# lucidrains/alphafold2

Measured on NVIDIA B200. Metric: evoformer_residue_pairs_per_sec, higher is better.
Workload: dtype bf16

## Files before the change

alphafold2_b200/csrc/api.cu:

```cuda
#include <cuda.h>
#include <cuda_runtime.h>
#include <cudaTypedefs.h>
#include <nvtx3/nvToolsExt.h>

#include <cstdarg>
#include <cstdio>
#include <cstdlib>
#include <cstring>
#include <vector>

#include "../../include/af2b200.h"
#include "attention_tc.cuh"
#include "chan2tok_tma.cuh"
#include "gemm_tc.cuh"
#include "ff_tc.cuh"
#include "proj_tc.cuh"
#include "simt_kernels.cuh"
#include "strict_kernels.cuh"
#include "glue_kernels.cuh"

using namespace af2;

namespace {

thread_local char g_err[512] = "";

int fail(int code, const char* fmt, ...) {
  va_list ap;
  va_start(ap, fmt);
  vsnprintf(g_err, sizeof(g_err), fmt, ap);
  va_end(ap);
  return code;
}

#define CUDA_OK(expr)                                                                            \
  do {                                                                                           \
    cudaError_t _e = (expr);                                                                     \
    if (_e != cudaSuccess) return fail(AF2_ERR_CUDA, "%s: %s (%s:%d)", #expr, cudaGetErrorString(_e), __FILE__, __LINE__); \
  } while (0)
#define AF2_TRY(expr)            \
  do {                           \
    int _r = (expr);             \
    if (_r != AF2_OK) return _r; \
  } while (0)

constexpr int MAX_DEVICES = 64;
int cur_dev() {
  int dev = 0;
  cudaGetDevice(&dev);
  return (dev >= 0 && dev < MAX_DEVICES) ? dev : 0;
}
int sm_count() {
  static int n[MAX_DEVICES] = {0};
  const int dev = cur_dev();
  if (n[dev] == 0) {
    cudaDeviceGetAttribute(&n[dev], cudaDevAttrMultiProcessorCount, dev);
    if (n[dev] <= 0) n[dev] = 148;
  }
  return n[dev];
}

int g_x_evict_last = 0;
inline int x_hint(long long tokens, int d) {
  const double mb = (double)tokens * d * 4 / 1e6;
  return (g_x_evict_last && mb >= 48.0 && mb <= 100.0) ? 1 : 0;
}

int g_pdl = 1;
template <class... KArgs, class... Args>
cudaError_t launch_pdl(void (*kern)(KArgs...), dim3 grid, dim3 block, size_t smem, cudaStream_t s, Args&&... args) {
  cudaLaunchConfig_t cfg;
  memset(&cfg, 0, sizeof(cfg));
  cfg.gridDim = grid; cfg.blockDim = block; cfg.dynamicSmemBytes = smem; cfg.stream = s;
  cudaLaunchAttribute at[1];
  at[0].id = cudaLaunchAttributeProgrammaticStreamSerialization;
  at[0].val.programmaticStreamSerializationAllowed = 1;
  cfg.attrs = at; cfg.numAttrs = g_pdl ? 1 : 0;
  return cudaLaunchKernelEx(&cfg, kern, static_cast<KArgs>(args)...);
}

struct NvtxRange {
  explicit NvtxRange(const char* name) { nvtxRangePushA(name); }
  ~NvtxRange() { nvtxRangePop(); }
};

enum KClass { KC_GEMM_LINEAR = 0, KC_GEMM_CHANNEL = 1, KC_ATTENTION = 2, KC_LAYERNORM = 3, KC_CHAN2TOK = 4, KC_MISC = 5, KC_COUNT = 6 };
struct ProfRec { cudaEvent_t a, b; int cls; double flops, bytes; };
unsigned long long g_launches = 0;
bool g_prof = false;
std::vector<ProfRec> g_recs;
std::vector<cudaEvent_t> g_pool;

cudaEvent_t prof_event() {
  if (!g_pool.empty()) { cudaEvent_t e = g_pool.back(); g_pool.pop_back(); return e; }
  cudaEvent_t e; cudaEventCreate(&e); return e;
}
struct ProfScope {
  cudaStream_t s; bool on; ProfRec r;
  ProfScope(cudaStream_t st, int cls, double flops, double bytes) : s(st), on(g_prof) {
    ++g_launches;
    if (on) { r.a = prof_event(); r.b = prof_event(); r.cls = cls; r.flops = flops; r.bytes = bytes; cudaEventRecord(r.a, s); }
  }
  ~ProfScope() { if (on) { cudaEventRecord(r.b, s); g_recs.push_back(r); } }
};

PFN_cuTensorMapEncodeTiled_v12000 encode_fn() {
  static PFN_cuTensorMapEncodeTiled_v12000 fn = nullptr;
  if (!fn) {
    void* p = nullptr;
    cudaDriverEntryPointQueryResult q;
    if (cudaGetDriverEntryPoint("cuTensorMapEncodeTiled", &p, cudaEnableDefault, &q) == cudaSuccess &&
        q == cudaDriverEntryPointSuccess)
      fn = reinterpret_cast<PFN_cuTensorMapEncodeTiled_v12000>(p);
  }
  return fn;
}

int make_tmap(CUtensorMap* m, const void* base, int rank, const unsigned long long* dims,
              const unsigned long long* strides_bytes, const unsigned* box, CUtensorMapSwizzle swz,
              CUtensorMapDataType dt = CU_TENSOR_MAP_DATA_TYPE_BFLOAT16,
              CUtensorMapL2promotion promo = CU_TENSOR_MAP_L2_PROMOTION_L2_256B) {
  auto fn = encode_fn();
  if (!fn) return fail(AF2_ERR_CUDA, "cuTensorMapEncodeTiled entry point not available");
  cuuint64_t gdim[5];
  cuuint64_t gstr[4];
  cuuint32_t bx[5], es[5];
  for (int i = 0; i < rank; ++i) {
    gdim[i] = dims[i];
    bx[i] = box[i];
    es[i] = 1;
  }
  for (int i = 0; i + 1 < rank; ++i) gstr[i] = strides_bytes[i];
  if (reinterpret_cast<uintptr_t>(base) & 15) return fail(AF2_ERR_BAD_ARG, "TMA base pointer not 16-byte aligned");
  for (int i = 0; i + 1 < rank; ++i)
    if (gstr[i] & 15) return fail(AF2_ERR_BAD_ARG, "TMA stride %d (%llu B) not a multiple of 16", i, (unsigned long long)gstr[i]);
  CUresult r = fn(m, dt, rank, const_cast<void*>(base), gdim, gstr, bx, es,
                  CU_TENSOR_MAP_INTERLEAVE_NONE, swz, promo,
                  CU_TENSOR_MAP_FLOAT_OOB_FILL_NONE);
  if (r != CUDA_SUCCESS) return fail(AF2_ERR_CUDA, "cuTensorMapEncodeTiled failed with CUresult %d", (int)r);
  return AF2_OK;
}

bool aligned16(const void* p) { return (reinterpret_cast<uintptr_t>(p) & 15) == 0; }
inline long long align_up(long long v, long long a) { return (v + a - 1) / a * a; }

struct Arena {
  char* base;
  long long size, off;
  bool ok;
  Arena(void* b, long long s) : base(static_cast<char*>(b)), size(s), off(0), ok(true) {}
  template <class T>
  T* take(long long count) {
    long long bytes = align_up(count * (long long)sizeof(T), 256);
    if (off + bytes > size) {
      ok = false;
      return nullptr;
    }
    T* p = reinterpret_cast<T*>(base + off);
    off += bytes;
    return p;
  }
};

struct GemmCall {
  const void* A; long long lda; long long a_batch;
  const void* Bm; long long ldb; long long b_batch;
  int M, N, K, batch;
  bool mn_major;
  int bn;
  int mode, act, layout, use_rowscale;
  void* out; long long ld_out; long long out_batch;
  const float* bias; const float* rowscale; const float* resid; long long ld_resid;
  int cm_inner, cm_pitch;
  int out_cols;
  int nseg; long long a_half, b_half;
  int a_pr, b_pr; long long a_piece, b_piece;
};

template <int BN, int STAGES, bool MN, int EK>
int launch_gemm_inst(const CUtensorMap& ta, const CUtensorMap& tb, const CUtensorMap& tc, const CUtensorMap& tr,
                     const GemmParams& p, cudaStream_t s) {
  using L = GemmSmem<BN, STAGES>;
  static bool configured[MAX_DEVICES] = {false};
  auto kern = gemm_tc_kernel<BN, STAGES, MN, EK>;
  if (!configured[cur_dev()]) {
    CUDA_OK(cudaFuncSetAttribute(kern, cudaFuncAttributeMaxDynamicSharedMemorySize, L::TOTAL));
    configured[cur_dev()] = true;
  }
  const int m_tiles = (p.M + GEMM_BM - 1) / GEMM_BM;
  const long long total = (long long)p.batch * m_tiles * p.num_ntiles;
  if (total <= 0) return AF2_OK;
  const int grid = (int)(total < sm_count() ? total : sm_count());
  const double flops = 2.0 * p.batch * (double)p.M * p.N * p.K;
  const double obytes = (p.tile.mode == EPI_STORE_BF16 ? 2.0 : (p.tile.mode == EPI_GATED_BF16 ? 1.0 : (p.tile.mode == EPI_RESID_F32 ? 8.0 : 4.0)));
  const double bytes = p.batch * ((double)p.M * p.K * 2 + (p.batch > 1 ? (double)p.N * p.K * 2 : 0) + (double)p.M * p.N * obytes) +
                       (p.batch > 1 ? 0 : (double)p.N * p.K * 2);
  ProfScope ps(s, p.batch > 1 ? KC_GEMM_CHANNEL : KC_GEMM_LINEAR, flops, bytes);
  CUDA_OK(launch_pdl(kern, dim3(grid), dim3(GEMM_THREADS), L::TOTAL, s, ta, tb, tc, tr, p));
  return AF2_OK;
}

int launch_gemm(const GemmCall& c, cudaStream_t s) {
  if (c.M <= 0 || c.N <= 0 || c.K <= 0 || c.batch <= 0) return AF2_OK;
  CUtensorMap ta, tb;
  const int BN = c.bn;
  if (c.nseg > 1) {
    const unsigned long long npl = c.nseg == 6 ? 3ull : 2ull;
    const unsigned long long ab = (unsigned long long)(c.batch > 1 ? c.a_batch : 0) * 2, bb_ = (unsigned long long)(c.batch > 1 ? c.b_batch : 0) * 2;
    if (!c.mn_major) {
      unsigned long long da[4] = {(unsigned long long)c.K, (unsigned long long)c.M, npl, (unsigned long long)c.batch};
      unsigned long long sa[3] = {(unsigned long long)c.lda * 2, (unsigned long long)c.a_half * 2, ab ? ab : (unsigned long long)c.a_half * 8};
      unsigned ba[4] = {64, 128, 1, 1};
      AF2_TRY(make_tmap(&ta, c.A, 4, da, sa, ba, CU_TENSOR_MAP_SWIZZLE_128B));
      unsigned long long db[4] = {(unsigned long long)c.K, (unsigned long long)c.N, npl, (unsigned long long)c.batch};
      unsigned long long sb[3] = {(unsigned long long)c.ldb * 2, (unsigned long long)c.b_half * 2, bb_ ? bb_ : (unsigned long long)c.b_half * 8};
      unsigned bx[4] = {64, (unsigned)BN, 1, 1};
      AF2_TRY(make_tmap(&tb, c.Bm, 4, db, sb, bx, CU_TENSOR_MAP_SWIZZLE_128B));
    } else {
      unsigned long long da[4] = {(unsigned long long)c.M, (unsigned long long)c.K, npl, (unsigned long long)c.batch};
      unsigned long long sa[3] = {(unsigned long long)c.lda * 2, (unsigned long long)c.a_half * 2, ab ? ab : (unsigned long long)c.a_half * 8};
      unsigned bx[4] = {64, 64, 1, 1};
      AF2_TRY(make_tmap(&ta, c.A, 4, da, sa, bx, CU_TENSOR_MAP_SWIZZLE_128B));
      unsigned long long db[4] = {(unsigned long long)c.N, (unsigned long long)c.K, npl, (unsigned long long)c.batch};
      unsigned long long sb[3] = {(unsigned long long)c.ldb * 2, (unsigned long long)c.b_half * 2, bb_ ? bb_ : (unsigned long long)c.b_half * 8};
      AF2_TRY(make_tmap(&tb, c.Bm, 4, db, sb, bx, CU_TENSOR_MAP_SWIZZLE_128B));
    }
  } else if (!c.mn_major) {
    unsigned long long da[3] = {(unsigned long long)c.K, (unsigned long long)c.M, (unsigned long long)c.batch};
    unsigned long long sa[2] = {(unsigned long long)c.lda * 2, (unsigned long long)(c.batch > 1 ? c.a_batch : c.lda * c.M) * 2};
    unsigned ba[3] = {64, 128, 1};
    AF2_TRY(make_tmap(&ta, c.A, 3, da, sa, ba, CU_TENSOR_MAP_SWIZZLE_128B));
    unsigned long long db[3] = {(unsigned long long)c.K, (unsigned long long)c.N, (unsigned long long)c.batch};
    unsigned long long sb[2] = {(unsigned long long)c.ldb * 2, (unsigned long long)(c.batch > 1 && c.b_batch ? c.b_batch : c.ldb * c.N) * 2};
    unsigned bb[3] = {64, (unsigned)BN, 1};
    AF2_TRY(make_tmap(&tb, c.Bm, 3, db, sb, bb, CU_TENSOR_MAP_SWIZZLE_128B));
  } else {
    unsigned long long da[3] = {(unsigned long long)c.M, (unsigned long long)c.K, (unsigned long long)c.batch};
    unsigned long long sa[2] = {(unsigned long long)c.lda * 2, (unsigned long long)(c.batch > 1 ? c.a_batch : c.lda * c.K) * 2};
    unsigned bx[3] = {64, 64, 1};
    AF2_TRY(make_tmap(&ta, c.A, 3, da, sa, bx, CU_TENSOR_MAP_SWIZZLE_128B));
    unsigned long long db[3] = {(unsigned long long)c.N, (unsigned long long)c.K, (unsigned long long)c.batch};
    unsigned long long sb[2] = {(unsigned long long)c.ldb * 2, (unsigned long long)(c.batch > 1 ? c.b_batch : c.ldb * c.K) * 2};
    AF2_TRY(make_tmap(&tb, c.Bm, 3, db, sb, bx, CU_TENSOR_MAP_SWIZZLE_128B));
  }
  if (c.nseg <= 1 && (c.a_pr > 0 || c.b_pr > 0)) {
    const unsigned long long bsa = (unsigned long long)(c.batch > 1 ? c.a_batch : c.lda) * 2, bsb = (unsigned long long)(c.batch > 1 ? c.b_batch : c.ldb) * 2;
    if (!c.mn_major) {
      if (c.a_pr > 0) {
        if (c.a_pr % 128 != 0) return fail(AF2_ERR_BAD_ARG, "gemm: gathered A pieces of %d rows (need a multiple of 128)", c.a_pr);
        unsigned long long da[4] = {(unsigned long long)c.K, (unsigned long long)c.a_pr, (unsigned long long)((c.M + c.a_pr - 1) / c.a_pr), (unsigned long long)c.batch};
        unsigned long long sa[3] = {(unsigned long long)c.lda * 2, (unsigned long long)c.a_piece * 2, bsa};
        unsigned ba[4] = {64, 128, 1, 1};
        AF2_TRY(make_tmap(&ta, c.A, 4, da, sa, ba, CU_TENSOR_MAP_SWIZZLE_128B));
      }
      if (c.b_pr > 0) {
        if (!((c.b_pr % BN) == 0 || (BN % c.b_pr) == 0) || c.b_pr % 8) return fail(AF2_ERR_BAD_ARG, "gemm: gathered B pieces of %d rows do not tile BN=%d", c.b_pr, BN);
        unsigned long long db[4] = {(unsigned long long)c.K, (unsigned long long)c.b_pr, (unsigned long long)((c.N + c.b_pr - 1) / c.b_pr), (unsigned long long)c.batch};
        unsigned long long sb[3] = {(unsigned long long)c.ldb * 2, (unsigned long long)c.b_piece * 2, bsb};
        unsigned bb[4] = {64, (unsigned)(c.b_pr >= BN ? BN : c.b_pr), (unsigned)(c.b_pr >= BN ? 1 : BN / c.b_pr), 1};
        AF2_TRY(make_tmap(&tb, c.Bm, 4, db, sb, bb, CU_TENSOR_MAP_SWIZZLE_128B));
      }
    } else {
      unsigned bx[4] = {64, 64, 1, 1};
      if (c.a_pr > 0) {
        if (c.a_pr % 64) return fail(AF2_ERR_BAD_ARG, "gemm: gathered MN-major A pieces of %d columns (need a multiple of 64)", c.a_pr);
        unsigned long long da[4] = {(unsigned long long)c.a_pr, (unsigned long long)c.K, (unsigned long long)((c.M + c.a_pr - 1) / c.a_pr), (unsigned long long)c.batch};
        unsigned long long sa[3] = {(unsigned long long)c.lda * 2, (unsigned long long)c.a_piece * 2, bsa};
        AF2_TRY(make_tmap(&ta, c.A, 4, da, sa, bx, CU_TENSOR_MAP_SWIZZLE_128B));
      }
      if (c.b_pr > 0) {
        if (c.b_pr % 64) return fail(AF2_ERR_BAD_ARG, "gemm: gathered MN-major B pieces of %d columns (need a multiple of 64)", c.b_pr);
        unsigned long long db[4] = {(unsigned long long)c.b_pr, (unsigned long long)c.K, (unsigned long long)((c.N + c.b_pr - 1) / c.b_pr), (unsigned long long)c.batch};
        unsigned long long sb[3] = {(unsigned long long)c.ldb * 2, (unsigned long long)c.b_piece * 2, bsb};
        AF2_TRY(make_tmap(&tb, c.Bm, 4, db, sb, bx, CU_TENSOR_MAP_SWIZZLE_128B));
      }
    }
  }
  GemmParams p;
  memset(&p, 0, sizeof(p));
  p.M = c.M; p.N = c.N; p.K = c.K; p.batch = c.batch; p.nseg = c.nseg > 1 ? c.nseg : 1;
  if (c.nseg <= 1) { p.a_pr = c.a_pr; p.b_pr = c.b_pr; }
  p.x_evict_last = (c.mode == EPI_RESID_F32) ? x_hint(c.M, c.N) : 0;
  p.num_ntiles = (c.N + BN - 1) / BN;
  p.out_cols = c.out_cols > 0 ? c.out_cols : ((c.mode == EPI_GATED_BF16) ? c.N / 2 : c.N);
  p.rowscale = c.rowscale; p.resid = c.resid; p.ld_resid = c.ld_resid;
  p.out_batch_stride = c.out_batch;
  p.cm_inner = c.cm_inner > 0 ? c.cm_inner : 1; p.cm_pitch = c.cm_pitch > 0 ? c.cm_pitch : 1;
  p.tile.mode = c.mode; p.tile.act = c.act; p.tile.layout = c.layout; p.tile.use_rowscale = c.use_rowscale;
  p.tile.out = c.out; p.tile.bias = c.bias; p.tile.ld = c.ld_out;
  const bool out_f32 = (c.mode == EPI_RESID_F32 || c.mode == EPI_STORE_F32);
  const int es = out_f32 ? 4 : 2;
  const int W = (c.mode == EPI_GATED_BF16) ? BN / 2 : BN;
  bool direct = false;
  if (!out_f32 && (W % 64) != 0) direct = true;
  if ((reinterpret_cast<uintptr_t>(c.out) & 15) != 0) direct = true;
  if (c.layout == LAYOUT_TOKEN) {
    if ((c.ld_out * es) % 16 != 0) direct = true;
    if (c.batch > 1 && (c.out_batch * es) % 16 != 0) direct = true;
  } else {
    if (c.cm_pitch != c.cm_inner || (c.ld_out * 2) % 16 != 0 || c.batch != 1 || out_f32) direct = true;
  }
  if (c.mode == EPI_RESID_F32 && ((c.ld_resid * 4) % 16 != 0 || (reinterpret_cast<uintptr_t>(c.resid) & 15) != 0)) direct = true;
  const bool resid_w = !direct && c.mode == EPI_RESID_F32 && BN == 256 && !c.mn_major && c.batch == 1 && c.N <= 256 &&
                       p.out_cols == 256;
  CUtensorMap tc = ta, tr = ta;
  if (!direct) {
    const CUtensorMapDataType dt = out_f32 ? CU_TENSOR_MAP_DATA_TYPE_FLOAT32 : CU_TENSOR_MAP_DATA_TYPE_BFLOAT16;
    if (c.layout == LAYOUT_TOKEN) {
      unsigned long long dc[3] = {(unsigned long long)p.out_cols, (unsigned long long)c.M, (unsigned long long)c.batch};
      unsigned long long sc[2] = {(unsigned long long)c.ld_out * es, (unsigned long long)(c.batch > 1 ? c.out_batch : c.ld_out * c.M) * es};
      unsigned bc[3] = {(unsigned)(out_f32 ? 32 : 64), (unsigned)(resid_w ? 32 : 128), 1};
      AF2_TRY(make_tmap(&tc, c.out, 3, dc, sc, bc, CU_TENSOR_MAP_SWIZZLE_128B, dt));
      if (c.mode == EPI_RESID_F32) {
        unsigned long long sr[2] = {(unsigned long long)c.ld_resid * 4, (unsigned long long)c.ld_resid * c.M * 4};
        AF2_TRY(make_tmap(&tr, c.resid, 3, dc, sr, bc, CU_TENSOR_MAP_SWIZZLE_128B, dt));
      }
    } else {
      unsigned long long dc[3] = {(unsigned long long)c.M, (unsigned long long)p.out_cols, 1ull};
      unsigned long long sc[2] = {(unsigned long long)c.ld_out * 2, (unsigned long long)c.ld_out * p.out_cols * 2};
      unsigned bc[3] = {64, 64, 1};
      AF2_TRY(make_tmap(&tc, c.out, 3, dc, sc, bc, CU_TENSOR_MAP_SWIZZLE_128B, dt));
    }
  }
  p.direct = direct ? 1 : 0;
  int ek = EK_GENERIC;
  if (!direct && BN == 256) {
    if (c.mode == EPI_STORE_BF16 && c.layout == LAYOUT_TOKEN && c.act == ACT_NONE && !c.use_rowscale) ek = EK_STORE_TOK;
    else if (c.mode == EPI_STORE_BF16 && c.layout == LAYOUT_TOKEN && c.act == ACT_SIGMOID && !c.use_rowscale) ek = EK_STORE_TOK_SIG;
    else if (c.mode == EPI_STORE_BF16 && c.layout == LAYOUT_CHANNEL && c.act == ACT_NONE) ek = EK_STORE_CH;
    else if (c.mode == EPI_GATED_BF16 && c.layout == LAYOUT_TOKEN && c.act == ACT_GELU && !c.use_rowscale) ek = EK_GATED_TOK_GELU;
    else if (c.mode == EPI_GATED_BF16 && c.layout == LAYOUT_CHANNEL && c.act == ACT_SIGMOID) ek = EK_GATED_CH_SIG;
    else if (c.mode == EPI_RESID_F32) ek = resid_w ? EK_RESID_F32_W : EK_RESID_F32;
    else if (c.mode == EPI_STORE_F32) ek = EK_STORE_F32;
  }
  if (c.mn_major) {
    if (BN == 256) {
      if (ek == EK_STORE_F32) return launch_gemm_inst<256, 3, true, EK_STORE_F32>(ta, tb, tc, tr, p, s);
      return launch_gemm_inst<256, 3, true, EK_GENERIC>(ta, tb, tc, tr, p, s);
    }
    if (BN == 128) return launch_gemm_inst<128, 4, true, EK_GENERIC>(ta, tb, tc, tr, p, s);
    return launch_gemm_inst<64, 6, true, EK_GENERIC>(ta, tb, tc, tr, p, s);
  }
  if (BN == 256) {
    switch (ek) {
      case EK_STORE_TOK: return launch_gemm_inst<256, 3, false, EK_STORE_TOK>(ta, tb, tc, tr, p, s);
      case EK_STORE_TOK_SIG: return launch_gemm_inst<256, 3, false, EK_STORE_TOK_SIG>(ta, tb, tc, tr, p, s);
      case EK_STORE_CH: return launch_gemm_inst<256, 3, false, EK_STORE_CH>(ta, tb, tc, tr, p, s);
      case EK_GATED_TOK_GELU: return launch_gemm_inst<256, 3, false, EK_GATED_TOK_GELU>(ta, tb, tc, tr, p, s);
      case EK_GATED_CH_SIG: return launch_gemm_inst<256, 3, false, EK_GATED_CH_SIG>(ta, tb, tc, tr, p, s);
      case EK_RESID_F32: return launch_gemm_inst<256, 3, false, EK_RESID_F32>(ta, tb, tc, tr, p, s);
      case EK_RESID_F32_W: return launch_gemm_inst<256, 3, false, EK_RESID_F32_W>(ta, tb, tc, tr, p, s);
      case EK_STORE_F32: return launch_gemm_inst<256, 3, false, EK_STORE_F32>(ta, tb, tc, tr, p, s);
      default: return launch_gemm_inst<256, 3, false, EK_GENERIC>(ta, tb, tc, tr, p, s);
    }
  }
  if (BN == 128) return launch_gemm_inst<128, 4, false, EK_GENERIC>(ta, tb, tc, tr, p, s);
  return launch_gemm_inst<64, 6, false, EK_GENERIC>(ta, tb, tc, tr, p, s);
}

int pick_bn(int n) { return n > 128 ? 256 : (n > 64 ? 128 : 64); }

GemmCall linear_call(const void* A, long long lda, const void* W, long long ldw, int M, int N, int K) {
  GemmCall c;
  memset(&c, 0, sizeof(c));
  c.A = A; c.lda = lda; c.Bm = W; c.ldb = ldw; c.M = M; c.N = N; c.K = K; c.batch = 1;
  c.mn_major = false; c.bn = pick_bn(N);
  return c;
}

int launch_layernorm(const LnParams& p, cudaStream_t s) {
  if (p.T <= 0) return AF2_OK;
  if (p.d % 4 != 0 || p.d > 1024) return fail(AF2_ERR_BAD_ARG, "LayerNorm: dim %d must be a multiple of 4 and <= 1024", p.d);
  const long long blocks_needed = (p.T + 7) / 8;
  const long long cap = (long long)sm_count() * 16;
  const int grid = (int)(blocks_needed < cap ? blocks_needed : cap);
  ProfScope ps(s, KC_LAYERNORM, 0.0, (double)p.T * p.d * (p.y ? 6.0 : 4.0) + (p.wb ? (double)p.T * p.heads * 2 : 0));
  if (p.d <= 128) layernorm_rows_kernel<1><<<grid, 256, 0, s>>>(p);
  else if (p.d <= 256) layernorm_rows_kernel<2><<<grid, 256, 0, s>>>(p);
  else if (p.d <= 512) layernorm_rows_kernel<4><<<grid, 256, 0, s>>>(p);
  else layernorm_rows_kernel<8><<<grid, 256, 0, s>>>(p);
  CUDA_OK(cudaGetLastError());
  return AF2_OK;
}

bool pair_bias_fast_ok(int d, int heads) { return d % 32 == 0 && d >= 32 && d <= 256 && heads <= 8; }
int launch_pair_bias(const float* x, long long T, int d, const float* wb, __nv_bfloat16* bias_out, int heads, long long bias_hs,
                     int n_inner, int pitch, cudaStream_t s, int transpose = 0) {
  if (T <= 0) return AF2_OK;
  PairBiasParams p;
  p.x = x; p.T = T; p.d = d; p.wb = wb; p.bias_out = bias_out; p.heads = heads; p.bias_hs = bias_hs; p.n_inner = n_inner; p.pitch = pitch;
  p.x_evict_last = x_hint(T, d);
  p.transpose = transpose;
  if (T > 0x7fffffffLL) return fail(AF2_ERR_BAD_ARG, "pair_bias: too many tokens");
  const bool mma = (d == 256 || d == 128);
  const long long need = mma ? (T + 127) / 128 : (T + 31) / 32;
  const long long cap = (long long)sm_count() * 3;
  const int grid = (int)(need < cap ? need : cap);
  ProfScope ps(s, KC_LAYERNORM, 0.0, (double)T * d * 4 + (double)T * heads * 2);
  if (mma && d == 256) CUDA_OK(launch_pdl(pair_bias_mma_kernel<16>, dim3(grid), dim3(256), 0, s, p));
  else if (mma) CUDA_OK(launch_pdl(pair_bias_mma_kernel<8>, dim3(grid), dim3(256), 0, s, p));
  else {
    switch (d / 32) {
      case 7: pair_bias_kernel<7><<<grid, 256, 0, s>>>(p); break;
      case 6: pair_bias_kernel<6><<<grid, 256, 0, s>>>(p); break;
      case 5: pair_bias_kernel<5><<<grid, 256, 0, s>>>(p); break;
      case 3: pair_bias_kernel<3><<<grid, 256, 0, s>>>(p); break;
      case 2: pair_bias_kernel<2><<<grid, 256, 0, s>>>(p); break;
      default: pair_bias_kernel<1><<<grid, 256, 0, s>>>(p); break;
    }
  }
  CUDA_OK(cudaGetLastError());
  return AF2_OK;
}

template <int D>
int launch_chan_to_token_tma(const ChanLnParams& p, long long T, cudaStream_t s) {
  using L = Chan2TokSmem<D>;
  static bool configured[MAX_DEVICES] = {false};
  auto kern = chan_to_token_tma_kernel<D>;
  if (!configured[cur_dev()]) {
    CUDA_OK(cudaFuncSetAttribute(kern, cudaFuncAttributeMaxDynamicSharedMemorySize, L::TOTAL));
    configured[cur_dev()] = true;
  }
  CUtensorMap tx, tg, ty;
  {
    unsigned long long dx[2] = {(unsigned long long)T, (unsigned long long)D};
    unsigned long long sx[1] = {(unsigned long long)p.chan_stride * 4};
    unsigned bx[2] = {C2T_TOK, (unsigned)D};
    AF2_TRY(make_tmap(&tx, p.src, 2, dx, sx, bx, CU_TENSOR_MAP_SWIZZLE_NONE, CU_TENSOR_MAP_DATA_TYPE_FLOAT32));
    unsigned long long dy[2] = {(unsigned long long)D, (unsigned long long)T};
    unsigned long long sy[1] = {(unsigned long long)D * 2};
    unsigned by[2] = {64, C2T_TOK};
    AF2_TRY(make_tmap(&ty, p.y, 2, dy, sy, by, CU_TENSOR_MAP_SWIZZLE_128B));
    if (p.mode == 0) AF2_TRY(make_tmap(&tg, p.gate, 2, dy, sy, by, CU_TENSOR_MAP_SWIZZLE_128B));
    else tg = ty;
  }
  Chan2TokParams q;
  q.T = T; q.mode = p.mode; q.gamma = p.gamma; q.beta = p.beta; q.scale = p.scale; q.scale_const = p.scale_const; q.eps = p.eps;
  const long long tiles = (T + C2T_TOK - 1) / C2T_TOK;
  const int grid = (int)(tiles < sm_count() ? tiles : sm_count());
  ProfScope ps(s, KC_CHAN2TOK, 0.0, (double)T * D * (p.mode == 0 ? 8.0 : 6.0));
  CUDA_OK(launch_pdl(kern, dim3(grid), dim3(L::THREADS), L::TOTAL, s, tx, tg, ty, q));
  return AF2_OK;
}

int g_c2t_tma = 1;
int g_attn_bias_t = 0;
int g_attn_ident_tmem = 1;
int g_attn_skip = 0;
int g_attn_k3 = 0;
int g_attn_headmajor = 0;
long long* g_attn_trace = nullptr;
int g_attn_l2pf = 0;
int g_attn_group = 1;
int g_gather_fused = 1;

int launch_chan_to_token(const ChanLnParams& p, cudaStream_t s) {
  const long long T = (long long)p.rows * p.n;
  if (g_c2t_tma && p.pitch == p.n && (p.d == 256 || p.d == 128) && (p.chan_stride % 4) == 0 && T > 0 && T < (1ll << 31) &&
      aligned16(p.src) && aligned16(p.y) && (p.mode != 0 || aligned16(p.gate))) {
    return p.d == 256 ? launch_chan_to_token_tma<256>(p, T, s) : launch_chan_to_token_tma<128>(p, T, s);
  }
  if (p.pitch == p.n && p.d % 64 == 0 && p.d <= 256 && (T % 4) == 0) {
    const size_t smem = (size_t)p.d * 64 * sizeof(float) + 8 * 64 * 2 * sizeof(float);
    static bool configured[MAX_DEVICES] = {false};
    if (!configured[cur_dev()]) {
      CUDA_OK(cudaFuncSetAttribute(chan_to_token_tile_kernel<32>, cudaFuncAttributeMaxDynamicSharedMemorySize, 256 * 64 * 4 + 4096));
      CUDA_OK(cudaFuncSetAttribute(chan_to_token_tile_kernel<24>, cudaFuncAttributeMaxDynamicSharedMemorySize, 192 * 64 * 4 + 4096));
      configured[cur_dev()] = true;
    }
    ProfScope ps(s, KC_CHAN2TOK, 0.0, (double)T * p.d * (p.mode == 0 ? 8.0 : 6.0));
    const unsigned grid = (unsigned)((T + 63) / 64);
    switch (p.d / 64) {
      case 4: chan_to_token_tile_kernel<32><<<grid, 512, smem, s>>>(p, T); break;
      case 3: chan_to_token_tile_kernel<24><<<grid, 512, smem, s>>>(p, T); break;
      case 2: chan_to_token_tile_kernel<16><<<grid, 512, smem, s>>>(p, T); break;
      default: chan_to_token_tile_kernel<8><<<grid, 512, smem, s>>>(p, T); break;
    }
    CUDA_OK(cudaGetLastError());
    return AF2_OK;
  }
  const size_t smem = (size_t)p.d * 33 * sizeof(float);
  static size_t configured[MAX_DEVICES] = {0};
  if (smem > 48 * 1024 && smem > configured[cur_dev()]) {
    CUDA_OK(cudaFuncSetAttribute(chan_to_token_kernel, cudaFuncAttributeMaxDynamicSharedMemorySize, (int)smem));
    configured[cur_dev()] = smem;
  }
  dim3 grid((p.n + 31) / 32, p.rows);
  ProfScope ps(s, KC_CHAN2TOK, 0.0, (double)p.rows * p.n * p.d * (p.mode == 0 ? 8.0 : 6.0));
  chan_to_token_kernel<<<grid, 256, smem, s>>>(p);
  CUDA_OK(cudaGetLastError());
  return AF2_OK;
}

template <int DH>
int launch_attention_inst(const CUtensorMap& tq, const CUtensorMap& tk, const CUtensorMap& tv, const CUtensorMap& tbias,
                          const CUtensorMap& tg, const CUtensorMap& to, const AttnParams& p, cudaStream_t s) {
  using L = AttnSmem<DH>;
  static bool configured[MAX_DEVICES] = {false};
  auto kern = attention_tc_kernel<DH>;
  if (!configured[cur_dev()]) {
    CUDA_OK(cudaFuncSetAttribute(kern, cudaFuncAttributeMaxDynamicSharedMemorySize, L::TOTAL));
    configured[cur_dev()] = true;
  }
  const int nqb = (p.n + 127) / 128;
  const long long items = (long long)nqb * p.heads * p.nbatch;
  if (items <= 0) return AF2_OK;
  int grid = (int)(items < sm_count() ? items : sm_count());
  if (nqb >= 2 && nqb <= 8 && g_attn_group) grid = grid / nqb * nqb;
  const double tokens = (double)p.n * p.nbatch;
  ProfScope ps(s, KC_ATTENTION, 4.0 * tokens * p.n * p.heads * DH,
               tokens * p.heads * DH * 2.0 * 5 + (p.has_bias ? (double)p.heads * p.n * p.n * 2 : 0));
  CUDA_OK(launch_pdl(kern, dim3(grid), dim3(ATTN_THREADS), L::TOTAL, s, tq, tk, tv, tbias, tg, to, p));
  return AF2_OK;
}

int launch_attention(const __nv_bfloat16* qkv, int heads, int dh, int n, int nbatch, long long tok_sb, long long tok_si,
                     const __nv_bfloat16* bias, int npad, const uint8_t* mask, const __nv_bfloat16* gate,
                     __nv_bfloat16* out, cudaStream_t s, const __nv_bfloat16* qkv_hm = nullptr, long long hm_tokens = 0, int bias_t = 0) {
  const long long I = (long long)heads * dh;
  const long long ld = 3 * I;
  CUtensorMap tq, tk, tv, tb, tg, to;
  unsigned long long dims[4] = {(unsigned long long)dh, (unsigned long long)n, (unsigned long long)heads, (unsigned long long)nbatch};
  unsigned long long str[3] = {(unsigned long long)(tok_si * ld * 2), (unsigned long long)(dh * 2), (unsigned long long)(tok_sb * ld * 2)};
  if (qkv_hm) {
    str[0] = (unsigned long long)(tok_si * dh * 2); str[1] = (unsigned long long)(hm_tokens * dh * 2); str[2] = (unsigned long long)(tok_sb * dh * 2);
  }
  unsigned box[4] = {(unsigned)dh, 128, 1, 1};
  const CUtensorMapSwizzle swz = (dh == 64) ? CU_TENSOR_MAP_SWIZZLE_128B : CU_TENSOR_MAP_SWIZZLE_64B;
  const CUtensorMapL2promotion promo = (dh == 64) ? CU_TENSOR_MAP_L2_PROMOTION_L2_128B : CU_TENSOR_MAP_L2_PROMOTION_L2_64B;
  const CUtensorMapDataType bf = CU_TENSOR_MAP_DATA_TYPE_BFLOAT16;
  if (qkv_hm) {
    const long long part = (long long)heads * hm_tokens * dh;
    AF2_TRY(make_tmap(&tq, qkv_hm, 4, dims, str, box, swz, bf, CU_TENSOR_MAP_L2_PROMOTION_L2_256B));
    AF2_TRY(make_tmap(&tk, qkv_hm + part, 4, dims, str, box, swz, bf, CU_TENSOR_MAP_L2_PROMOTION_L2_256B));
    AF2_TRY(make_tmap(&tv, qkv_hm + 2 * part, 4, dims, str, box, swz, bf, CU_TENSOR_MAP_L2_PROMOTION_L2_256B));
  } else {
    AF2_TRY(make_tmap(&tq, qkv, 4, dims, str, box, swz, bf, promo));
    AF2_TRY(make_tmap(&tk, qkv + I, 4, dims, str, box, swz, bf, promo));
    AF2_TRY(make_tmap(&tv, qkv + 2 * I, 4, dims, str, box, swz, bf, promo));
  }
  unsigned long long gstr[3] = {(unsigned long long)(tok_si * I * 2), (unsigned long long)(dh * 2), (unsigned long long)(tok_sb * I * 2)};
  AF2_TRY(make_tmap(&tg, gate, 4, dims, gstr, box, swz, bf, promo));
  unsigned obox[4] = {(unsigned)dh, 32, 1, 1};
  AF2_TRY(make_tmap(&to, out, 4, dims, gstr, obox, swz));
  if (bias) {
    unsigned long long bd[3] = {(unsigned long long)npad, (unsigned long long)n, (unsigned long long)heads};
    unsigned long long bs[2] = {(unsigned long long)npad * 2, (unsigned long long)n * npad * 2};
    unsigned bb[3] = {64, 128, 1};
    AF2_TRY(make_tmap(&tb, bias, 3, bd, bs, bb, CU_TENSOR_MAP_SWIZZLE_128B));
  } else {
    tb = tq;
  }
  AttnParams p;
  memset(&p, 0, sizeof(p));
  p.n = n; p.heads = heads; p.nbatch = nbatch; p.has_bias = bias != nullptr;
  p.mask = mask; p.mask_sb = tok_sb; p.mask_si = tok_si;
  p.gate = gate; p.out = out; p.tok_sb = tok_sb; p.tok_si = tok_si; p.ld_gate = I; p.ld_out = I;
  p.l2_prefetch = g_attn_l2pf;
  p.k_stages3 = g_attn_k3;
  p.dbg_skip = g_attn_skip;
  p.ident_tmem = g_attn_ident_tmem;
  p.bias_t = bias_t;
  p.trace = g_attn_trace;
  if (dh == 64) return launch_attention_inst<64>(tq, tk, tv, tb, tg, to, p, s);
  if (dh == 32) return launch_attention_inst<32>(tq, tk, tv, tb, tg, to, p, s);
  return fail(AF2_ERR_BAD_ARG, "attention: dim_head %d unsupported (32 or 64)", dh);
}

#include "proj_launch.inl"

int g_ff_fused = 1;

bool ff_fused_ok(const af2_ff_weights* w, int d, int hidden) {
  return g_ff_fused && g_proj_ctas == 2 && w->w_cat && w->w_ext && w->bn == 256 && (d == 128 || d == 256) &&
         hidden % FF_CHUNK == 0 && aligned16(w->w2) && aligned16(w->b2);
}

int launch_ff_fused(const af2_ff_weights* w, float* x, long long T, int d, int hidden, cudaStream_t s) {
  if (T <= 0) return AF2_OK;
  if (!aligned16(x)) return fail(AF2_ERR_BAD_ARG, "feed_forward: x not 16-byte aligned");
  using L = FfSmem;
  static bool configured_dev[MAX_DEVICES] = {false};
  static int max_clusters_dev[MAX_DEVICES] = {0};
  int& max_clusters = max_clusters_dev[cur_dev()];
  if (!configured_dev[cur_dev()]) {
    CUDA_OK(cudaFuncSetAttribute(ff_tc_kernel, cudaFuncAttributeMaxDynamicSharedMemorySize, L::TOTAL));
    cudaLaunchConfig_t qc;
    memset(&qc, 0, sizeof(qc));
    qc.gridDim = dim3(sm_count(), 1, 1); qc.blockDim = dim3(FF_THREADS, 1, 1); qc.dynamicSmemBytes = L::TOTAL;
    cudaLaunchAttribute qa[1];
    qa[0].id = cudaLaunchAttributeClusterDimension; qa[0].val.clusterDim.x = 2; qa[0].val.clusterDim.y = 1; qa[0].val.clusterDim.z = 1;
    qc.attrs = qa; qc.numAttrs = 1;
    int nc = 0;
    if (cudaOccupancyMaxActiveClusters(&nc, ff_tc_kernel, &qc) != cudaSuccess || nc <= 0) { cudaGetLastError(); nc = sm_count() / 2; }
    max_clusters = nc < sm_count() / 2 ? nc : sm_count() / 2;
    configured_dev[cur_dev()] = true;
  }
  const int n1p = (hidden + 127) / 128 * 256;
  CUtensorMap tw1, tb1, tw2, tx;
  {
    unsigned long long dw[2] = {(unsigned long long)d, (unsigned long long)n1p};
    unsigned long long sw[1] = {(unsigned long long)d * 2};
    unsigned bw[2] = {64, 64};
    AF2_TRY(make_tmap(&tw1, w->w_cat, 2, dw, sw, bw, CU_TENSOR_MAP_SWIZZLE_128B));
    unsigned long long dx[2] = {16ull, (unsigned long long)n1p};
    unsigned long long sx[1] = {32ull};
    unsigned bx[2] = {16, 64};
    AF2_TRY(make_tmap(&tb1, w->w_ext, 2, dx, sx, bx, CU_TENSOR_MAP_SWIZZLE_32B));
    unsigned long long d2[2] = {(unsigned long long)hidden, (unsigned long long)d};
    unsigned long long s2[1] = {(unsigned long long)hidden * 2};
    unsigned b2[2] = {64, (unsigned)(d / 2)};
    AF2_TRY(make_tmap(&tw2, w->w2, 2, d2, s2, b2, CU_TENSOR_MAP_SWIZZLE_128B));
    unsigned long long dxr[2] = {(unsigned long long)d, (unsigned long long)T};
    unsigned long long sxr[1] = {(unsigned long long)d * 4};
    unsigned bxr[2] = {32, 32};
    AF2_TRY(make_tmap(&tx, x, 2, dxr, sxr, bxr, CU_TENSOR_MAP_SWIZZLE_128B, CU_TENSOR_MAP_DATA_TYPE_FLOAT32));
  }
  FfParams p;
  memset(&p, 0, sizeof(p));
  p.x = x; p.b2 = w->b2; p.T = T; p.d = d; p.hidden = hidden; p.inv_d = 1.0f / (float)d; p.eps = 1e-5f;
  p.m_units = (int)((T + 255) / 256);
  const int clusters = p.m_units < max_clusters ? p.m_units : max_clusters;
  const double flops = 2.0 * T * (double)d * hidden * 3;
  const double bytes = (double)T * d * 8 + (double)n1p * d * 2 + (double)d * hidden * 2;
  ProfScope ps(s, KC_GEMM_LINEAR, flops, bytes);
  cudaLaunchConfig_t cfg;
  memset(&cfg, 0, sizeof(cfg));
  cfg.gridDim = dim3(clusters * 2, 1, 1); cfg.blockDim = dim3(FF_THREADS, 1, 1); cfg.dynamicSmemBytes = L::TOTAL; cfg.stream = s;
  cudaLaunchAttribute at[2];
  at[0].id = cudaLaunchAttributeClusterDimension; at[0].val.clusterDim.x = 2; at[0].val.clusterDim.y = 1; at[0].val.clusterDim.z = 1;
  at[1].id = cudaLaunchAttributeProgrammaticStreamSerialization; at[1].val.programmaticStreamSerializationAllowed = 1;
  cfg.attrs = at; cfg.numAttrs = g_pdl ? 2 : 1;
  CUDA_OK(cudaLaunchKernelEx(&cfg, ff_tc_kernel, tw1, tb1, tw2, tx, p));
  return AF2_OK;
}

int launch_outer_scale(const uint8_t* mask, float* scale, uint32_t* words, int row0, int rows, int S, int N, float eps, cudaStream_t s);

int ew_grid(long long n) {
  long long b = (n + 255) / 256;
  long long cap = (long long)sm_count() * 8;
  return (int)(b < cap ? (b > 0 ? b : 1) : cap);
}

int launch_outer_scale(const uint8_t* mask, float* scale, uint32_t* words, int row0, int rows, int S, int N, float eps, cudaStream_t s) {
  const long long T = (long long)rows * N;
  if (T <= 0) return AF2_OK;
  const int nw = (S + 31) / 32;
  const size_t smem = (size_t)nw * N * 4;
  ProfScope ps(s, KC_MISC, 0.0, 0.0);
  if (words && smem <= 160 * 1024) {
    static size_t configured[MAX_DEVICES] = {0};
    if (smem > 48 * 1024 && smem > configured[cur_dev()]) {
      CUDA_OK(cudaFuncSetAttribute(outer_scale_bits_kernel, cudaFuncAttributeMaxDynamicSharedMemorySize, (int)smem));
      configured[cur_dev()] = smem;
    }
    mask_pack_bits_kernel<<<ew_grid((long long)nw * N), 256, 0, s>>>(mask, words, S, N);
    CUDA_OK(cudaGetLastError());
    const long long need = (T + 255) / 256;
    const int grid = (int)(need < sm_count() ? need : sm_count());
    outer_scale_bits_kernel<<<grid, 256, smem, s>>>(words, scale, row0, rows, S, N, eps);
  } else {
    outer_scale_rows_kernel<<<ew_grid(T), 256, 0, s>>>(mask, scale, row0, rows, S, N, eps);
  }
  CUDA_OK(cudaGetLastError());
  return AF2_OK;
}

}

extern "C" {

const char* af2_last_error(void) { return g_err; }
int af2_abi_version(void) { return 2; }

unsigned long long af2_launch_count(void) { return g_launches; }

void af2_profile_enable(int on) {
  g_prof = on != 0;
  if (g_prof) {
    for (auto& r : g_recs) { g_pool.push_back(r.a); g_pool.push_back(r.b); }
    g_recs.clear();
  }
}

long long af2_profile_read(int cls, double* ms, double* flops, double* bytes) {
  cudaDeviceSynchronize();
  double t = 0, f = 0, b = 0;
  long long n = 0;
  for (auto& r : g_recs) {
    if (r.cls != cls) continue;
    float e = 0.f;
    if (cudaEventElapsedTime(&e, r.a, r.b) == cudaSuccess) t += e;
    f += r.flops; b += r.bytes; ++n;
  }
  if (ms) *ms = t;
  if (flops) *flops = f;
  if (bytes) *bytes = b;
  return n;
}

int af2_debug_proj_trace(long long* out) {
  if (!g_proj_trace) return fail(AF2_ERR_BAD_ARG, "projection trace not enabled (AF2_PROJ_TRACE=1)");
  CUDA_OK(cudaDeviceSynchronize());
  CUDA_OK(cudaMemcpy(out, g_proj_trace, 2048 * sizeof(long long), cudaMemcpyDeviceToHost));
  return AF2_OK;
}

int af2_debug_attn_trace(long long* out) {
  if (!g_attn_trace) return fail(AF2_ERR_BAD_ARG, "attention trace not enabled (AF2_ATTN_TRACE=1)");
  CUDA_OK(cudaDeviceSynchronize());
  CUDA_OK(cudaMemcpy(out, g_attn_trace, 1024 * sizeof(long long), cudaMemcpyDeviceToHost));
  CUDA_OK(cudaMemset(g_attn_trace, 0, 1024 * sizeof(long long)));
  return AF2_OK;
}

void af2_set_proj_mode(int ctas) { g_proj_ctas = ctas < 0 ? 2 : (ctas > 2 ? 2 : ctas); }
void af2_set_ff_fused(int on) { g_ff_fused = on != 0; }

int af2_check_device(void) {
  if (const char* e = getenv("AF2_PROJ_CTAS")) af2_set_proj_mode(atoi(e));
  if (const char* e = getenv("AF2_FF_FUSED")) af2_set_ff_fused(atoi(e));
  if (const char* e = getenv("AF2_C2T_TMA")) g_c2t_tma = atoi(e) != 0;
  if (const char* e = getenv("AF2_PROJ_PRODTILES")) g_proj_prod_tiles = atof(e);
  if (const char* e = getenv("AF2_PROJ_BALANCE")) g_proj_balance = atoi(e) != 0;
  if (const char* e = getenv("AF2_PROJ_WIDE")) g_proj_wide = atoi(e) != 0;
  if (const char* e = getenv("AF2_PROJ_L2PF")) g_proj_l2pf = atoi(e) != 0;
  if (const char* e = getenv("AF2_GATHER_FUSED")) g_gather_fused = atoi(e) != 0;
  if (const char* e = getenv("AF2_ATTN_GROUP")) g_attn_group = atoi(e) != 0;
  if (const char* e = getenv("AF2_ATTN_L2PF")) g_attn_l2pf = atoi(e) != 0;
  if (const char* e = getenv("AF2_ATTN_HEADMAJOR")) g_attn_headmajor = atoi(e) != 0;
  if (const char* e = getenv("AF2_ATTN_K3")) g_attn_k3 = atoi(e) != 0;
  if (const char* e = getenv("AF2_ATTN_SKIP")) g_attn_skip = atoi(e);
  if (const char* e = getenv("AF2_ATTN_IDENT_TMEM")) g_attn_ident_tmem = atoi(e) != 0;
  if (const char* e = getenv("AF2_ATTN_BIAS_T")) g_attn_bias_t = atoi(e) != 0;
  if (const char* e = getenv("AF2_ATTN_TRACE")) {
    if (atoi(e) != 0 && !g_attn_trace) {
      if (cudaMalloc(&g_attn_trace, 1024 * sizeof(long long)) != cudaSuccess) g_attn_trace = nullptr;
      else cudaMemset(g_attn_trace, 0, 1024 * sizeof(long long));
    }
  }
  if (const char* e = getenv("AF2_X_EVICT_LAST")) g_x_evict_last = atoi(e) != 0;
  if (const char* e = getenv("AF2_PDL")) g_pdl = atoi(e) != 0;
  if (const char* e = getenv("AF2_PROJ_TRACE")) {
    if (atoi(e) != 0 && !g_proj_trace) {
      if (cudaMalloc(&g_proj_trace, 2048 * sizeof(long long)) != cudaSuccess) g_proj_trace = nullptr;
      else cudaMemset(g_proj_trace, 0, 2048 * sizeof(long long));
    }
  }
  int dev = 0;
  if (cudaGetDevice(&dev) != cudaSuccess) return fail(AF2_ERR_CUDA, "no CUDA device");
  int major = 0;
  cudaDeviceGetAttribute(&major, cudaDevAttrComputeCapabilityMajor, dev);
  if (major != 10) return fail(AF2_ERR_UNSUPPORTED_DEVICE, "libaf2b200 is built for sm_100a only; device has compute capability %d.x", major);
  return AF2_OK;
}

long long af2_feed_forward_workspace(long long tokens, int d, int hidden) {
  return align_up(tokens * d * 2, 256) + align_up(tokens * hidden * 2, 256) + 1024;
}

int af2_feed_forward(const af2_ff_weights* w, float* x, long long tokens, int d, int hidden, void* workspace,
                     long long workspace_bytes, af2_stream_t stream) {
  NvtxRange nvtx_("af2_feed_forward");
  cudaStream_t s = static_cast<cudaStream_t>(stream);
  if (!w || !x) return fail(AF2_ERR_BAD_ARG, "feed_forward: null argument");
  if (d % 8 || hidden % 8) return fail(AF2_ERR_BAD_ARG, "feed_forward: d=%d and hidden=%d must be multiples of 8", d, hidden);
  if (tokens > 0x7fffffffLL) return fail(AF2_ERR_BAD_ARG, "feed_forward: too many tokens");
  if (ff_fused_ok(w, d, hidden)) return launch_ff_fused(w, x, tokens, d, hidden, s);
  Arena ar(workspace, workspace_bytes);
  __nv_bfloat16* xn = ar.take<__nv_bfloat16>(tokens * d);
  __nv_bfloat16* hbuf = ar.take<__nv_bfloat16>(tokens * hidden);
  if (!ar.ok) return fail(AF2_ERR_WORKSPACE, "feed_forward: workspace too small");
  const int half = w->bn / 2;
  const int n1p = (hidden + half - 1) / half * w->bn;
  if (g_proj_ctas > 0 && w->w_cat && w->bn == 256 && proj_dim_ok(d)) {
    ProjCall pc;
    memset(&pc, 0, sizeof(pc));
    pc.x = x; pc.T = tokens; pc.d = d;
    pc.w_cat = w->w_cat; pc.w_ext = w->w_ext; pc.nseg = 1;
    pc.seg[0] = ProjOut{n1p / 256, EK_GATED_TOK_GELU, hidden, hbuf, hidden};
    AF2_TRY(launch_proj(pc, s));
  } else {
    LnParams lp;
    memset(&lp, 0, sizeof(lp));
    lp.x = x; lp.gamma = w->ln_gamma; lp.beta = w->ln_beta; lp.y = xn; lp.T = tokens; lp.d = d; lp.eps = 1e-5f;
    AF2_TRY(launch_layernorm(lp, s));
    GemmCall c1 = linear_call(xn, d, w->w1, d, (int)tokens, n1p, d);
    c1.bn = w->bn; c1.mode = EPI_GATED_BF16; c1.act = ACT_GELU; c1.layout = LAYOUT_TOKEN;
    c1.out = hbuf; c1.ld_out = hidden; c1.bias = w->b1; c1.out_cols = hidden;
    AF2_TRY(launch_gemm(c1, s));
  }
  GemmCall c2 = linear_call(hbuf, hidden, w->w2, hidden, (int)tokens, d, hidden);
  c2.mode = EPI_RESID_F32; c2.out = x; c2.ld_out = d; c2.bias = w->b2; c2.resid = x; c2.ld_resid = d;
  AF2_TRY(launch_gemm(c2, s));
  return AF2_OK;
}

long long af2_axial_attention_workspace(int B, int h, int wdim, int d, int heads, int dim_head, int row_attn) {
  const long long T = (long long)B * h * wdim, I = (long long)heads * dim_head;
  const int n = row_attn ? wdim : h;
  const long long npad = align_up(n, 8);
  return align_up(T * d * 2, 256) + 2 * align_up(T * 3 * I * 2, 256) + 2 * align_up(T * I * 2, 256) +
         align_up((long long)B * heads * n * npad * 2, 256) + 1024;
}

static int axial_attention_impl(const af2_attn_weights* w, float* x, const float* edges, const void* pre_bias,
                                const unsigned char* mask, int B, int h, int wdim, int d, int heads, int dim_head,
                                int row_attn, void* workspace, long long workspace_bytes, af2_stream_t stream, int tied = 0) {
  NvtxRange nvtx_(row_attn ? "af2_axial_attention(row)" : "af2_axial_attention(col)");
  cudaStream_t s = static_cast<cudaStream_t>(stream);
  if (!w || !x) return fail(AF2_ERR_BAD_ARG, "axial_attention: null argument");
  if (dim_head != 32 && dim_head != 64) return fail(AF2_ERR_BAD_ARG, "axial_attention: dim_head %d unsupported (32 or 64)", dim_head);
  if (d % 8) return fail(AF2_ERR_BAD_ARG, "axial_attention: dim %d must be a multiple of 8", d);
  const long long T = (long long)B * h * wdim, I = (long long)heads * dim_head;
  if (T > 0x7fffffffLL) return fail(AF2_ERR_BAD_ARG, "axial_attention: too many tokens");
  const int n = row_attn ? wdim : h;
  const int nb = row_attn ? h : wdim;
  const int npad = (int)align_up(n, 8);
  const bool has_bias = pre_bias != nullptr || (edges != nullptr && w->w_edge != nullptr);
  Arena ar(workspace, workspace_bytes);
  __nv_bfloat16* xn = ar.take<__nv_bfloat16>(T * d);
  __nv_bfloat16* qkv = ar.take<__nv_bfloat16>(T * 3 * I);
  __nv_bfloat16* gate = ar.take<__nv_bfloat16>(T * I);
  __nv_bfloat16* og = ar.take<__nv_bfloat16>(T * I);
  __nv_bfloat16* bias = ar.take<__nv_bfloat16>((long long)B * heads * n * npad);
  __nv_bfloat16* qkv_hm = ar.take<__nv_bfloat16>(T * 3 * I);
  if (!ar.ok) return fail(AF2_ERR_WORKSPACE, "axial_attention: workspace too small");
  if (pre_bias) bias = const_cast<__nv_bfloat16*>(static_cast<const __nv_bfloat16*>(pre_bias));

  const bool fused_proj = g_proj_ctas > 0 && w->w_cat && proj_dim_ok(d) && (I % 8) == 0;
  LnParams lp;
  memset(&lp, 0, sizeof(lp));
  lp.x = x; lp.gamma = w->ln_gamma; lp.beta = w->ln_beta; lp.y = xn; lp.T = T; lp.d = d; lp.eps = 1e-5f;
  const bool fuse_bias = has_bias && !pre_bias && edges == x && B == 1;
  const bool bias_t = g_attn_bias_t && has_bias && !pre_bias && pair_bias_fast_ok(d, heads) && !(fuse_bias && !fused_proj);
  if (has_bias && !pre_bias && npad != n) CUDA_OK(cudaMemsetAsync(bias, 0, (size_t)B * heads * n * npad * 2, s));
  if (fuse_bias) {
    lp.wb = w->w_edge; lp.bias_out = bias; lp.heads = heads; lp.bias_hs = (long long)n * npad; lp.n_inner = n; lp.pitch = npad;
  }
  if (!fused_proj) {
    AF2_TRY(launch_layernorm(lp, s));
  } else if (fuse_bias) {
    if (pair_bias_fast_ok(d, heads)) {
      AF2_TRY(launch_pair_bias(x, T, d, w->w_edge, bias, heads, (long long)n * npad, n, npad, s, bias_t ? 1 : 0));
    } else {
      lp.y = nullptr;
      AF2_TRY(launch_layernorm(lp, s));
    }
  }
  if (has_bias && !fuse_bias && !pre_bias && pair_bias_fast_ok(d, heads)) {
    for (int b = 0; b < B; ++b)
      AF2_TRY(launch_pair_bias(edges + (long long)b * n * n * d, (long long)n * n, d, w->w_edge, bias + (long long)b * heads * n * npad,
                               heads, (long long)n * npad, n, npad, s, bias_t ? 1 : 0));
  } else if (has_bias && !fuse_bias && !pre_bias) {
    for (int b = 0; b < B; ++b) {
      LnParams bp;
      memset(&bp, 0, sizeof(bp));
      bp.x = edges + (long long)b * n * n * d; bp.T = (long long)n * n; bp.d = d; bp.eps = 1e-5f;
      bp.wb = w->w_edge; bp.bias_out = bias + (long long)b * heads * n * npad; bp.heads = heads;
      bp.bias_hs = (long long)n * npad; bp.n_inner = n; bp.pitch = npad;
      AF2_TRY(launch_layernorm(bp, s));
    }
  }
  if (fused_proj) {
    ProjCall pc;
    memset(&pc, 0, sizeof(pc));
    pc.x = x; pc.T = T; pc.d = d;
    pc.w_cat = w->w_cat; pc.w_ext = w->w_ext; pc.nseg = 2;
    pc.seg[0] = ProjOut{(int)((3 * I + 255) / 256), EK_STORE_TOK, (int)(3 * I), qkv, 3 * I};
    pc.seg[1] = ProjOut{(int)((I + 255) / 256), EK_STORE_TOK_SIG, (int)I, gate, I};
    AF2_TRY(launch_proj(pc, s));
  } else {
    GemmCall cq = linear_call(xn, d, w->w_qkv, d, (int)T, (int)(3 * I), d);
    cq.mode = EPI_STORE_BF16; cq.layout = LAYOUT_TOKEN; cq.out = qkv; cq.ld_out = 3 * I;
    AF2_TRY(launch_gemm(cq, s));
    GemmCall cg = linear_call(xn, d, w->w_gate, d, (int)T, (int)I, d);
    cg.mode = EPI_STORE_BF16; cg.act = ACT_SIGMOID; cg.layout = LAYOUT_TOKEN; cg.out = gate; cg.ld_out = I; cg.bias = w->b_gate;
    AF2_TRY(launch_gemm(cg, s));
  }
  const long long tok_sb = row_attn ? wdim : 1, tok_si = row_attn ? 1 : wdim;
  for (int b = 0; b < B; ++b) {
    const long long t0 = (long long)b * h * wdim;
    if (tied) {
      ProfScope ps(s, KC_MISC, 0.0, 0.0);
      tie_queries_kernel<__nv_bfloat16><<<ew_grid((long long)n * I), 256, 0, s>>>(qkv + t0 * 3 * I, 3 * I, (int)I, n, nb, tok_sb, tok_si);
      CUDA_OK(cudaGetLastError());
    }
    const long long Tb = (long long)h * wdim;
    if (g_attn_headmajor && dim_head % 8 == 0) {
      ProfScope ps(s, KC_MISC, 0.0, 0.0);
      qkv_to_headmajor_kernel<<<ew_grid(Tb * 3 * I / 8), 256, 0, s>>>(reinterpret_cast<const uint4*>(qkv + t0 * 3 * I),
                                                                        reinterpret_cast<uint4*>(qkv_hm + t0 * 3 * I), Tb, (int)(3 * I), dim_head);
      CUDA_OK(cudaGetLastError());
    }
    AF2_TRY(launch_attention(qkv + t0 * 3 * I, heads, dim_head, n, nb, tok_sb, tok_si,
                             has_bias ? bias + (long long)b * heads * n * npad : nullptr, npad,
                             mask ? mask + t0 : nullptr, gate + t0 * I, og + t0 * I, s,
                             (g_attn_headmajor && dim_head % 8 == 0) ? qkv_hm + t0 * 3 * I : nullptr, Tb, bias_t ? 1 : 0));
  }
  GemmCall co = linear_call(og, I, w->w_out, I, (int)T, d, (int)I);
  co.mode = EPI_RESID_F32; co.out = x; co.ld_out = d; co.bias = w->b_out; co.resid = x; co.ld_resid = d;
  AF2_TRY(launch_gemm(co, s));
  return AF2_OK;
}

long long af2_triangle_multiply_workspace(int B, int N, int d) {
  const long long T = (long long)B * N * N;
  const long long np8 = align_up(N, 8), np4 = align_up(N, 4);
  return 3 * align_up(T * d * 2, 256)
         + 2 * align_up((long long)d * B * N * np8 * 2, 256)
         + align_up((long long)d * B * N * np4 * 4, 256)
         + align_up(T * 4, 256) + 1024;
}

int af2_triangle_multiply(const af2_trimul_weights* w, float* x, const unsigned char* mask, int B, int N, int d,
                          int ingoing, void* workspace, long long workspace_bytes, af2_stream_t stream) {
  NvtxRange nvtx_("af2_triangle_multiply");
  cudaStream_t s = static_cast<cudaStream_t>(stream);
  if (!w || !x) return fail(AF2_ERR_BAD_ARG, "triangle_multiply: null argument");
  if (d % 32) return fail(AF2_ERR_BAD_ARG, "triangle_multiply: dim %d must be a multiple of 32", d);
  const long long T = (long long)B * N * N;
  if (T > 0x7fffffffLL) return fail(AF2_ERR_BAD_ARG, "triangle_multiply: too many tokens");
  const int np8 = (int)align_up(N, 8), np4 = (int)align_up(N, 4);
  const long long cs_lr = (long long)B * N * np8;
  const long long cs_o = (long long)B * N * np4;
  Arena ar(workspace, workspace_bytes);
  __nv_bfloat16* xn = ar.take<__nv_bfloat16>(T * d);
  __nv_bfloat16* gate = ar.take<__nv_bfloat16>(T * d);
  __nv_bfloat16* tn = ar.take<__nv_bfloat16>(T * d);
  __nv_bfloat16* Lc = ar.take<__nv_bfloat16>(d * cs_lr);
  __nv_bfloat16* Rc = ar.take<__nv_bfloat16>(d * cs_lr);
  float* Oc = ar.take<float>(d * cs_o);
  float* maskf = ar.take<float>(T);
  if (!ar.ok) return fail(AF2_ERR_WORKSPACE, "triangle_multiply: workspace too small");

  const bool fused_front = g_proj_ctas > 0 && w->w_cat && w->bn == 256 && proj_dim_ok(d) && np8 == N;
  if (fused_front) {
    ProjCall pc;
    memset(&pc, 0, sizeof(pc));
    pc.x = x; pc.T = T; pc.d = d;
    pc.w_cat = w->w_cat; pc.w_ext = w->w_ext; pc.rowmask = mask; pc.nseg = 3;
    const int tl = (d + 127) / 128;
    pc.seg[0] = ProjOut{tl, EK_GATED_CH_SIG, d, Lc, cs_lr};
    pc.seg[1] = ProjOut{tl, EK_GATED_CH_SIG, d, Rc, cs_lr};
    pc.seg[2] = ProjOut{(d + 255) / 256, EK_STORE_TOK_SIG, d, gate, (long long)d};
    AF2_TRY(launch_proj(pc, s));
  }
  LnParams lp;
  memset(&lp, 0, sizeof(lp));
  lp.x = x; lp.gamma = w->ln_gamma; lp.beta = w->ln_beta; lp.y = xn; lp.T = T; lp.d = d; lp.eps = 1e-5f;
  if (!fused_front) AF2_TRY(launch_layernorm(lp, s));
  if (mask && !fused_front) {
    { ProfScope ps(s, KC_MISC, 0.0, 0.0); mask_to_float_kernel<<<ew_grid(T), 256, 0, s>>>(mask, maskf, T); }
    CUDA_OK(cudaGetLastError());
  }
  if (np8 != N) {
    CUDA_OK(cudaMemsetAsync(Lc, 0, (size_t)d * cs_lr * 2, s));
    CUDA_OK(cudaMemsetAsync(Rc, 0, (size_t)d * cs_lr * 2, s));
  }
  const int half = w->bn / 2;
  const int npk = (d + half - 1) / half * w->bn;
  for (int side = 0; side < 2 && !fused_front; ++side) {
    GemmCall c = linear_call(xn, d, side ? w->w_right : w->w_left, d, (int)T, npk, d);
    c.bn = w->bn; c.mode = EPI_GATED_BF16; c.act = ACT_SIGMOID; c.layout = LAYOUT_CHANNEL;
    c.out = side ? Rc : Lc; c.ld_out = cs_lr; c.bias = side ? w->b_right : w->b_left;
    c.use_rowscale = mask != nullptr; c.rowscale = maskf; c.cm_inner = N; c.cm_pitch = np8; c.out_cols = d;
    AF2_TRY(launch_gemm(c, s));
  }
  GemmCall cg = linear_call(xn, d, w->w_ogate, d, (int)T, d, d);
  cg.mode = EPI_STORE_BF16; cg.act = ACT_SIGMOID; cg.layout = LAYOUT_TOKEN; cg.out = gate; cg.ld_out = d; cg.bias = w->b_ogate;
  if (!fused_front) AF2_TRY(launch_gemm(cg, s));
  for (int b = 0; b < B; ++b) {
    GemmCall c;
    memset(&c, 0, sizeof(c));
    const long long boff = (long long)b * N * np8;
    if (!ingoing) {
      c.A = Lc + boff; c.Bm = Rc + boff; c.mn_major = false;
    } else {
      c.A = Rc + boff; c.Bm = Lc + boff; c.mn_major = true;
    }
    c.lda = np8; c.ldb = np8; c.a_batch = cs_lr; c.b_batch = cs_lr;
    c.M = N; c.N = N; c.K = N; c.batch = d; c.bn = pick_bn(N);
    c.mode = EPI_STORE_F32; c.layout = LAYOUT_TOKEN; c.out = Oc + (long long)b * N * np4; c.ld_out = np4; c.out_batch = cs_o;
    AF2_TRY(launch_gemm(c, s));
  }
  ChanLnParams cp;
  memset(&cp, 0, sizeof(cp));
  cp.src = Oc; cp.chan_stride = cs_o; cp.pitch = np4; cp.rows = B * N; cp.n = N; cp.d = d; cp.mode = 0;
  cp.gamma = w->on_gamma; cp.beta = w->on_beta; cp.gate = gate; cp.eps = 1e-5f; cp.y = tn;
  AF2_TRY(launch_chan_to_token(cp, s));
  GemmCall co = linear_call(tn, d, w->w_out, d, (int)T, d, d);
  co.mode = EPI_RESID_F32; co.out = x; co.ld_out = d; co.bias = w->b_out; co.resid = x; co.ld_resid = d;
  AF2_TRY(launch_gemm(co, s));
  return AF2_OK;
}

long long af2_outer_mean_workspace(int B, int S, int N, int d) {
  const long long Tm = (long long)B * S * N, Tx = (long long)B * N * N;
  const long long np8 = align_up(N, 8), np4 = align_up(N, 4);
  return align_up(Tm * d * 2, 256) + align_up((long long)2 * d * B * S * np8 * 2, 256) +
         align_up((long long)d * B * N * np4 * 4, 256) + align_up(Tx * d * 2, 256) + align_up(Tm * 4, 256) +
         align_up(Tx * 4, 256) + align_up((long long)((S + 31) / 32) * N * 4, 256) + 1024;
}

int af2_outer_mean(const af2_outer_weights* w, float* x, const float* m, const unsigned char* msa_mask, int B, int S,
                   int N, int d, float eps, void* workspace, long long workspace_bytes, af2_stream_t stream) {
  NvtxRange nvtx_("af2_outer_mean");
  cudaStream_t s = static_cast<cudaStream_t>(stream);
  if (!w || !x || !m) return fail(AF2_ERR_BAD_ARG, "outer_mean: null argument");
  if (d % 32) return fail(AF2_ERR_BAD_ARG, "outer_mean: dim %d must be a multiple of 32", d);
  const long long Tm = (long long)B * S * N, Tx = (long long)B * N * N;
  if (Tm > 0x7fffffffLL || Tx > 0x7fffffffLL) return fail(AF2_ERR_BAD_ARG, "outer_mean: too many tokens");
  const int np8 = (int)align_up(N, 8), np4 = (int)align_up(N, 4);
  const long long cs_lr = (long long)B * S * np8, cs_o = (long long)B * N * np4;
  Arena ar(workspace, workspace_bytes);
  __nv_bfloat16* mn = ar.take<__nv_bfloat16>(Tm * d);
  __nv_bfloat16* LRc = ar.take<__nv_bfloat16>(2LL * d * cs_lr);
  float* Oc = ar.take<float>(d * cs_o);
  __nv_bfloat16* tn = ar.take<__nv_bfloat16>(Tx * d);
  float* maskf = ar.take<float>(Tm);
  float* scale = ar.take<float>(Tx);
  uint32_t* mwords = ar.take<uint32_t>((long long)((S + 31) / 32) * N);
  if (!ar.ok) return fail(AF2_ERR_WORKSPACE, "outer_mean: workspace too small");

  const bool fused_front = g_proj_ctas > 0 && w->w_cat && proj_dim_ok(d) && np8 == N;
  LnParams lp;
  memset(&lp, 0, sizeof(lp));
  lp.x = m; lp.gamma = w->ln_gamma; lp.beta = w->ln_beta; lp.y = mn; lp.T = Tm; lp.d = d; lp.eps = 1e-5f;
  if (!fused_front) AF2_TRY(launch_layernorm(lp, s));
  if (msa_mask) {
    if (!fused_front) { ProfScope ps(s, KC_MISC, 0.0, 0.0); mask_to_float_kernel<<<ew_grid(Tm), 256, 0, s>>>(msa_mask, maskf, Tm); }
    CUDA_OK(cudaGetLastError());
    for (int b = 0; b < B; ++b)
      AF2_TRY(launch_outer_scale(msa_mask + (long long)b * S * N, scale + (long long)b * N * N, mwords, 0, N, S, N, eps, s));
  }
  if (np8 != N) CUDA_OK(cudaMemsetAsync(LRc, 0, (size_t)2 * d * cs_lr * 2, s));
  if (fused_front) {
    ProjCall pc;
    memset(&pc, 0, sizeof(pc));
    pc.x = m; pc.T = Tm; pc.d = d;
    pc.w_cat = w->w_cat; pc.w_ext = w->w_ext; pc.rowmask = msa_mask; pc.nseg = 1;
    pc.seg[0] = ProjOut{(2 * d + 255) / 256, EK_STORE_CH, 2 * d, LRc, cs_lr};
    AF2_TRY(launch_proj(pc, s));
  } else {
    GemmCall c = linear_call(mn, d, w->w_lr, d, (int)Tm, 2 * d, d);
    c.mode = EPI_STORE_BF16; c.layout = LAYOUT_CHANNEL; c.out = LRc; c.ld_out = cs_lr; c.bias = w->b_lr;
    c.use_rowscale = msa_mask != nullptr; c.rowscale = maskf; c.cm_inner = N; c.cm_pitch = np8;
    AF2_TRY(launch_gemm(c, s));
  }
  for (int b = 0; b < B; ++b) {
    GemmCall g;
    memset(&g, 0, sizeof(g));
    g.A = LRc + (long long)b * S * np8; g.Bm = LRc + (long long)d * cs_lr + (long long)b * S * np8;
    g.mn_major = true; g.lda = np8; g.ldb = np8; g.a_batch = cs_lr; g.b_batch = cs_lr;
    g.M = N; g.N = N; g.K = S; g.batch = d; g.bn = pick_bn(N);
    g.mode = EPI_STORE_F32; g.layout = LAYOUT_TOKEN; g.out = Oc + (long long)b * N * np4; g.ld_out = np4; g.out_batch = cs_o;
    AF2_TRY(launch_gemm(g, s));
  }
  ChanLnParams cp;
  memset(&cp, 0, sizeof(cp));
  cp.src = Oc; cp.chan_stride = cs_o; cp.pitch = np4; cp.rows = B * N; cp.n = N; cp.d = d; cp.mode = 1;
  cp.scale = msa_mask ? scale : nullptr; cp.scale_const = 1.0f / (float)S; cp.y = tn;
  AF2_TRY(launch_chan_to_token(cp, s));
  GemmCall co = linear_call(tn, d, w->w_out, d, (int)Tx, d, d);
  co.mode = EPI_RESID_F32; co.out = x; co.ld_out = d; co.bias = w->b_out; co.resid = x; co.ld_resid = d;
  AF2_TRY(launch_gemm(co, s));
  return AF2_OK;
}


int af2_axial_attention(const af2_attn_weights* w, float* x, const float* edges, const unsigned char* mask, int B,
                        int h, int wdim, int d, int heads, int dim_head, int row_attn, void* workspace,
                        long long workspace_bytes, af2_stream_t stream) {
  return axial_attention_impl(w, x, edges, nullptr, mask, B, h, wdim, d, heads, dim_head, row_attn, workspace,
                              workspace_bytes, stream);
}

int af2_axial_attention_ex(const af2_attn_weights* w, float* x, const float* edges, const unsigned char* mask, int B,
                           int h, int wdim, int d, int heads, int dim_head, int row_attn, int flags, void* workspace,
                           long long workspace_bytes, af2_stream_t stream) {
  return axial_attention_impl(w, x, edges, nullptr, mask, B, h, wdim, d, heads, dim_head, row_attn, workspace,
                              workspace_bytes, stream, flags & 1);
}

int af2_axial_attention_prebias(const af2_attn_weights* w, float* x, const void* bias_bf16, const unsigned char* mask,
                                int B, int h, int wdim, int d, int heads, int dim_head, int row_attn, void* workspace,
                                long long workspace_bytes, af2_stream_t stream) {
  return axial_attention_impl(w, x, nullptr, bias_bf16, mask, B, h, wdim, d, heads, dim_head, row_attn, workspace,
                              workspace_bytes, stream);
}

int af2_pair_bias(const float* x_rows, const float* w_edge, void* bias_out, int rows, int n, int d, int heads,
                  af2_stream_t stream) {
  NvtxRange nvtx_("af2_pair_bias");
  cudaStream_t s = static_cast<cudaStream_t>(stream);
  if (!x_rows || !w_edge || !bias_out) return fail(AF2_ERR_BAD_ARG, "pair_bias: null argument");
  const int npad = (int)align_up(n, 8);
  if (pair_bias_fast_ok(d, heads))
    return launch_pair_bias(x_rows, (long long)rows * n, d, w_edge, static_cast<__nv_bfloat16*>(bias_out), heads, (long long)rows * npad,
                            n, npad, s);
  LnParams bp;
  memset(&bp, 0, sizeof(bp));
  bp.x = x_rows; bp.T = (long long)rows * n; bp.d = d; bp.eps = 1e-5f;
  bp.wb = w_edge; bp.bias_out = static_cast<__nv_bfloat16*>(bias_out); bp.heads = heads;
  bp.bias_hs = (long long)rows * npad; bp.n_inner = n; bp.pitch = npad;
  return launch_layernorm(bp, s);
}

long long af2_triangle_project_workspace(long long tokens, int d) {
  return align_up(tokens * d * 2, 256) + align_up(tokens * 4, 256) + 1024;
}

int af2_triangle_project(const af2_trimul_weights* w, const float* x, const unsigned char* mask, long long tokens,
                         int inner, int d, void* Lc, void* Rc, long long chan_stride, void* gate, void* workspace,
                         long long workspace_bytes, af2_stream_t stream) {
  NvtxRange nvtx_("af2_triangle_project");
  cudaStream_t s = static_cast<cudaStream_t>(stream);
  if (!w || !x || !Lc || !Rc || !gate) return fail(AF2_ERR_BAD_ARG, "triangle_project: null argument");
  if (d % 32) return fail(AF2_ERR_BAD_ARG, "triangle_project: dim %d must be a multiple of 32", d);
  if (tokens % inner) return fail(AF2_ERR_BAD_ARG, "triangle_project: tokens must be a multiple of inner");
  const int pitch = (int)align_up(inner, 8);
  Arena ar(workspace, workspace_bytes);
  __nv_bfloat16* xn = ar.take<__nv_bfloat16>(tokens * d);
  float* maskf = ar.take<float>(tokens);
  if (!ar.ok) return fail(AF2_ERR_WORKSPACE, "triangle_project: workspace too small");
  if (g_proj_ctas > 0 && w->w_cat && w->bn == 256 && proj_dim_ok(d) && pitch == inner) {
    ProjCall pc;
    memset(&pc, 0, sizeof(pc));
    pc.x = x; pc.T = tokens; pc.d = d;
    pc.w_cat = w->w_cat; pc.w_ext = w->w_ext; pc.rowmask = mask; pc.nseg = 3;
    const int tl = (d + 127) / 128;
    pc.seg[0] = ProjOut{tl, EK_GATED_CH_SIG, d, Lc, chan_stride};
    pc.seg[1] = ProjOut{tl, EK_GATED_CH_SIG, d, Rc, chan_stride};
    pc.seg[2] = ProjOut{(d + 255) / 256, EK_STORE_TOK_SIG, d, gate, (long long)d};
    return launch_proj(pc, s);
  }
  LnParams lp;
  memset(&lp, 0, sizeof(lp));
  lp.x = x; lp.gamma = w->ln_gamma; lp.beta = w->ln_beta; lp.y = xn; lp.T = tokens; lp.d = d; lp.eps = 1e-5f;
  AF2_TRY(launch_layernorm(lp, s));
  if (mask) {
    { ProfScope ps(s, KC_MISC, 0.0, 0.0); mask_to_float_kernel<<<ew_grid(tokens), 256, 0, s>>>(mask, maskf, tokens); }
    CUDA_OK(cudaGetLastError());
  }
  if (pitch != inner) {
    CUDA_OK(cudaMemsetAsync(Lc, 0, (size_t)d * chan_stride * 2, s));
    CUDA_OK(cudaMemsetAsync(Rc, 0, (size_t)d * chan_stride * 2, s));
  }
  const int half = w->bn / 2;
  const int npk = (d + half - 1) / half * w->bn;
  for (int side = 0; side < 2; ++side) {
    GemmCall c = linear_call(xn, d, side ? w->w_right : w->w_left, d, (int)tokens, npk, d);
    c.bn = w->bn; c.mode = EPI_GATED_BF16; c.act = ACT_SIGMOID; c.layout = LAYOUT_CHANNEL;
    c.out = side ? Rc : Lc; c.ld_out = chan_stride; c.bias = side ? w->b_right : w->b_left;
    c.use_rowscale = mask != nullptr; c.rowscale = maskf; c.cm_inner = inner; c.cm_pitch = pitch; c.out_cols = d;
    AF2_TRY(launch_gemm(c, s));
  }
  GemmCall cg = linear_call(xn, d, w->w_ogate, d, (int)tokens, d, d);
  cg.mode = EPI_STORE_BF16; cg.act = ACT_SIGMOID; cg.layout = LAYOUT_TOKEN; cg.out = gate; cg.ld_out = d; cg.bias = w->b_ogate;
  AF2_TRY(launch_gemm(cg, s));
  return AF2_OK;
}

long long af2_triangle_contract_workspace(int rows, int cols, int d) {
  return align_up((long long)d * rows * align_up(cols, 4) * 4, 256) + align_up((long long)rows * cols * d * 2, 256) + 1024;
}

int af2_triangle_contract(const af2_trimul_weights* w, float* x, const void* Lc, long long cs_l, const void* Rg,
                          long long cs_r, long long piece_stride, int pieces, const void* gate, int rows, int cols,
                          int K, int d, int ingoing, void* workspace, long long workspace_bytes, af2_stream_t stream) {
  NvtxRange nvtx_("af2_triangle_contract");
  cudaStream_t s = static_cast<cudaStream_t>(stream);
  if (!w || !x || !Lc || !Rg || !gate || pieces < 1) return fail(AF2_ERR_BAD_ARG, "triangle_contract: bad argument");
  if ((!ingoing && cols % pieces) || (ingoing && rows % pieces)) return fail(AF2_ERR_BAD_ARG, "triangle_contract: pieces must divide the gathered axis");
  const long long T = (long long)rows * cols;
  const int cp4 = (int)align_up(cols, 4);
  const long long cs_o = (long long)rows * cp4;
  Arena ar(workspace, workspace_bytes);
  float* Oc = ar.take<float>(d * cs_o);
  __nv_bfloat16* tn = ar.take<__nv_bfloat16>(T * d);
  if (!ar.ok) return fail(AF2_ERR_WORKSPACE, "triangle_contract: workspace too small");
  const __nv_bfloat16* L = static_cast<const __nv_bfloat16*>(Lc);
  const __nv_bfloat16* R = static_cast<const __nv_bfloat16*>(Rg);
  bool fused_pieces = false;
  if (pieces > 1 && g_gather_fused) {
    GemmCall c;
    memset(&c, 0, sizeof(c));
    c.batch = d; c.K = K; c.mode = EPI_STORE_F32; c.layout = LAYOUT_TOKEN; c.ld_out = cp4; c.out_batch = cs_o; c.out = Oc;
    if (!ingoing) {
      const int pc = cols / pieces, bn = pick_bn(cols);
      if (pc % 8 == 0 && (pc % bn == 0 || bn % pc == 0)) {
        c.A = L; c.lda = align_up(K, 8); c.a_batch = cs_l;
        c.Bm = R; c.ldb = align_up(K, 8); c.b_batch = cs_r; c.b_pr = pc; c.b_piece = piece_stride;
        c.mn_major = false; c.M = rows; c.N = cols; c.bn = bn;
        fused_pieces = true;
      }
    } else {
      const int pr = rows / pieces;
      if (pr % 64 == 0) {
        c.A = R; c.lda = align_up(pr, 8); c.a_batch = cs_r; c.a_pr = pr; c.a_piece = piece_stride;
        c.Bm = L; c.ldb = align_up(cols, 8); c.b_batch = cs_l;
        c.mn_major = true; c.M = rows; c.N = cols; c.bn = pick_bn(cols);
        fused_pieces = true;
      }
    }
    if (fused_pieces) AF2_TRY(launch_gemm(c, s));
  }
  for (int p = 0; p < pieces && !fused_pieces; ++p) {
    GemmCall c;
    memset(&c, 0, sizeof(c));
    c.batch = d; c.K = K; c.mode = EPI_STORE_F32; c.layout = LAYOUT_TOKEN; c.ld_out = cp4; c.out_batch = cs_o;
    if (!ingoing) {
      const int pc = cols / pieces;
      c.A = L; c.lda = align_up(K, 8); c.a_batch = cs_l;
      c.Bm = R + p * piece_stride; c.ldb = align_up(K, 8); c.b_batch = cs_r;
      c.mn_major = false; c.M = rows; c.N = pc; c.bn = pick_bn(pc);
      c.out = Oc + (long long)p * pc;
    } else {
      const int pr = rows / pieces;
      c.A = R + p * piece_stride; c.lda = align_up(pr, 8); c.a_batch = cs_r;
      c.Bm = L; c.ldb = align_up(cols, 8); c.b_batch = cs_l;
      c.mn_major = true; c.M = pr; c.N = cols; c.bn = pick_bn(cols);
      c.out = Oc + (long long)p * pr * cp4;
    }
    AF2_TRY(launch_gemm(c, s));
  }
  ChanLnParams cp;
  memset(&cp, 0, sizeof(cp));
  cp.src = Oc; cp.chan_stride = cs_o; cp.pitch = cp4; cp.rows = rows; cp.n = cols; cp.d = d; cp.mode = 0;
  cp.gamma = w->on_gamma; cp.beta = w->on_beta; cp.gate = static_cast<const __nv_bfloat16*>(gate); cp.eps = 1e-5f; cp.y = tn;
  AF2_TRY(launch_chan_to_token(cp, s));
  GemmCall co = linear_call(tn, d, w->w_out, d, (int)T, d, d);
  co.mode = EPI_RESID_F32; co.out = x; co.ld_out = d; co.bias = w->b_out; co.resid = x; co.ld_resid = d;
  AF2_TRY(launch_gemm(co, s));
  return AF2_OK;
}

long long af2_outer_project_workspace(long long tokens, int d) {
  return align_up(tokens * d * 2, 256) + align_up(tokens * 4, 256) + 1024;
}

int af2_outer_project(const af2_outer_weights* w, const float* m, const unsigned char* msa_mask, long long tokens,
                      int inner, int d, void* LRc, long long chan_stride, void* workspace, long long workspace_bytes,
                      af2_stream_t stream) {
  NvtxRange nvtx_("af2_outer_project");
  cudaStream_t s = static_cast<cudaStream_t>(stream);
  if (!w || !m || !LRc) return fail(AF2_ERR_BAD_ARG, "outer_project: null argument");
  if (d % 32) return fail(AF2_ERR_BAD_ARG, "outer_project: dim %d must be a multiple of 32", d);
  const int pitch = (int)align_up(inner, 8);
  Arena ar(workspace, workspace_bytes);
  __nv_bfloat16* mn = ar.take<__nv_bfloat16>(tokens * d);
  float* maskf = ar.take<float>(tokens);
  if (!ar.ok) return fail(AF2_ERR_WORKSPACE, "outer_project: workspace too small");
  if (g_proj_ctas > 0 && w->w_cat && proj_dim_ok(d) && pitch == inner) {
    ProjCall pc;
    memset(&pc, 0, sizeof(pc));
    pc.x = m; pc.T = tokens; pc.d = d;
    pc.w_cat = w->w_cat; pc.w_ext = w->w_ext; pc.rowmask = msa_mask; pc.nseg = 1;
    pc.seg[0] = ProjOut{(2 * d + 255) / 256, EK_STORE_CH, 2 * d, LRc, chan_stride};
    return launch_proj(pc, s);
  }
  LnParams lp;
  memset(&lp, 0, sizeof(lp));
  lp.x = m; lp.gamma = w->ln_gamma; lp.beta = w->ln_beta; lp.y = mn; lp.T = tokens; lp.d = d; lp.eps = 1e-5f;
  AF2_TRY(launch_layernorm(lp, s));
  if (msa_mask) {
    { ProfScope ps(s, KC_MISC, 0.0, 0.0); mask_to_float_kernel<<<ew_grid(tokens), 256, 0, s>>>(msa_mask, maskf, tokens); }
    CUDA_OK(cudaGetLastError());
  }
  if (pitch != inner) CUDA_OK(cudaMemsetAsync(LRc, 0, (size_t)2 * d * chan_stride * 2, s));
  GemmCall c = linear_call(mn, d, w->w_lr, d, (int)tokens, 2 * d, d);
  c.mode = EPI_STORE_BF16; c.layout = LAYOUT_CHANNEL; c.out = LRc; c.ld_out = chan_stride; c.bias = w->b_lr;
  c.use_rowscale = msa_mask != nullptr; c.rowscale = maskf; c.cm_inner = inner; c.cm_pitch = pitch;
  AF2_TRY(launch_gemm(c, s));
  return AF2_OK;
}

long long af2_outer_contract_workspace(int rows, int N, int d) {
  return align_up((long long)d * rows * align_up(N, 4) * 4, 256) + align_up((long long)rows * N * d * 2, 256) +
         align_up((long long)rows * N * 4, 256) + align_up((long long)N * 4096 / 8, 256) + 1024;
}

int af2_outer_contract(const af2_outer_weights* w, float* x, const void* Lc, long long cs_l, const void* Rg,
                       long long cs_r, long long piece_stride, int pieces, const unsigned char* msa_mask_full,
                       int row0, int rows, int N, int S, int d, float eps, void* workspace, long long workspace_bytes,
                       af2_stream_t stream) {
  NvtxRange nvtx_("af2_outer_contract");
  cudaStream_t s = static_cast<cudaStream_t>(stream);
  if (!w || !x || !Lc || !Rg || pieces < 1 || N % pieces) return fail(AF2_ERR_BAD_ARG, "outer_contract: bad argument");
  const long long T = (long long)rows * N;
  const int np4 = (int)align_up(N, 4);
  const long long cs_o = (long long)rows * np4;
  Arena ar(workspace, workspace_bytes);
  float* Oc = ar.take<float>(d * cs_o);
  __nv_bfloat16* tn = ar.take<__nv_bfloat16>(T * d);
  float* scale = ar.take<float>(T);
  uint32_t* mwords = (S <= 4096) ? ar.take<uint32_t>((long long)((S + 31) / 32) * N) : nullptr;
  if (!ar.ok) return fail(AF2_ERR_WORKSPACE, "outer_contract: workspace too small");
  if (msa_mask_full) AF2_TRY(launch_outer_scale(msa_mask_full, scale, mwords, row0, rows, S, N, eps, s));
  const __nv_bfloat16* L = static_cast<const __nv_bfloat16*>(Lc);
  const __nv_bfloat16* R = static_cast<const __nv_bfloat16*>(Rg);
  const int pc = N / pieces;
  const bool fused_pieces = pieces > 1 && g_gather_fused && pc % 64 == 0;
  if (fused_pieces) {
    GemmCall g;
    memset(&g, 0, sizeof(g));
    g.A = L; g.lda = align_up(rows, 8); g.a_batch = cs_l;
    g.Bm = R; g.ldb = align_up(pc, 8); g.b_batch = cs_r; g.b_pr = pc; g.b_piece = piece_stride;
    g.mn_major = true; g.M = rows; g.N = N; g.K = S; g.batch = d; g.bn = pick_bn(N);
    g.mode = EPI_STORE_F32; g.layout = LAYOUT_TOKEN; g.out = Oc; g.ld_out = np4; g.out_batch = cs_o;
    AF2_TRY(launch_gemm(g, s));
  }
  for (int p = 0; p < pieces && !fused_pieces; ++p) {
    GemmCall g;
    memset(&g, 0, sizeof(g));
    g.A = L; g.lda = align_up(rows, 8); g.a_batch = cs_l;
    g.Bm = R + p * piece_stride; g.ldb = align_up(pc, 8); g.b_batch = cs_r;
    g.mn_major = true; g.M = rows; g.N = pc; g.K = S; g.batch = d; g.bn = pick_bn(pc);
    g.mode = EPI_STORE_F32; g.layout = LAYOUT_TOKEN; g.out = Oc + (long long)p * pc; g.ld_out = np4; g.out_batch = cs_o;
    AF2_TRY(launch_gemm(g, s));
  }
  ChanLnParams cp;
  memset(&cp, 0, sizeof(cp));
  cp.src = Oc; cp.chan_stride = cs_o; cp.pitch = np4; cp.rows = rows; cp.n = N; cp.d = d; cp.mode = 1;
  cp.scale = msa_mask_full ? scale : nullptr; cp.scale_const = 1.0f / (float)S; cp.y = tn;
  AF2_TRY(launch_chan_to_token(cp, s));
  GemmCall co = linear_call(tn, d, w->w_out, d, (int)T, d, d);
  co.mode = EPI_RESID_F32; co.out = x; co.ld_out = d; co.bias = w->b_out; co.resid = x; co.ld_resid = d;
  AF2_TRY(launch_gemm(co, s));
  return AF2_OK;
}

int af2_rotary(const float* x, const float* sin_, const float* cos_, float* y, int b, int h, int n, int dh, int rot,
               int sincos_batch, af2_stream_t stream) {
  NvtxRange nvtx_("af2_rotary");
  cudaStream_t s = static_cast<cudaStream_t>(stream);
  if (dh % 2 || rot % 2 || rot > dh) return fail(AF2_ERR_BAD_ARG, "rotary: dh=%d rot=%d must be even, rot <= dh", dh, rot);
  const long long pairs = (long long)b * h * n * (dh / 2);
  if (pairs == 0) return AF2_OK;
  { ProfScope ps(s, KC_MISC, 0.0, 0.0); rotary_kernel<<<ew_grid(pairs), 256, 0, s>>>(x, sin_, cos_, y, b, h, n, dh, rot, sincos_batch); }
  CUDA_OK(cudaGetLastError());
  return AF2_OK;
}

int af2_layernorm_bf16(const float* x, const float* gamma, const float* beta, void* y_bf16, long long T, int d,
                       float eps, af2_stream_t stream) {
  LnParams lp;
  memset(&lp, 0, sizeof(lp));
  lp.x = x; lp.gamma = gamma; lp.beta = beta; lp.y = static_cast<__nv_bfloat16*>(y_bf16); lp.T = T; lp.d = d; lp.eps = eps;
  return launch_layernorm(lp, static_cast<cudaStream_t>(stream));
}

int af2_gemm_bf16_f32(const void* A, long long lda, long long a_batch, const void* Bm, long long ldb, long long b_batch,
                      float* C, long long ldc, long long c_batch, int M, int N, int K, int batch, int mn_major,
                      af2_stream_t stream) {
  GemmCall c;
  memset(&c, 0, sizeof(c));
  c.A = A; c.lda = lda; c.a_batch = a_batch; c.Bm = Bm; c.ldb = ldb; c.b_batch = b_batch;
  c.M = M; c.N = N; c.K = K; c.batch = batch; c.mn_major = mn_major != 0; c.bn = pick_bn(N);
  c.mode = EPI_STORE_F32; c.layout = LAYOUT_TOKEN; c.out = C; c.ld_out = ldc; c.out_batch = c_batch;
  return launch_gemm(c, static_cast<cudaStream_t>(stream));
}

}

#include "strict_api.inl"
#include "peer_api.inl"
```

alphafold2_b200/csrc/attention_tc.cuh:

```cuda
#pragma once
#include "common.cuh"

#ifndef AF2_ATTN_POLY_EXP
#define AF2_ATTN_POLY_EXP 0
#endif

namespace af2 {

struct AttnParams {
  int n;
  int heads;
  int nbatch;
  int has_bias;
  const uint8_t* mask;
  long long mask_sb, mask_si;
  const __nv_bfloat16* gate;
  __nv_bfloat16* out;
  long long tok_sb, tok_si;
  long long ld_gate, ld_out;
  long long* trace;
  int bias_t;
  int ident_tmem;
  int dbg_skip;
  int k_stages3;
  int l2_prefetch;
};

constexpr int ATTN_PF_DIST = 4;
constexpr int ATTN_NSPLIT = 4;
constexpr int ATTN_SM_WARPS = 4 * ATTN_NSPLIT;
constexpr int ATTN_W_KEYMASK = 2 + ATTN_SM_WARPS;
constexpr int ATTN_W_VPROD = ATTN_W_KEYMASK + 1;
constexpr int ATTN_W_EPI = ATTN_W_VPROD + 1;
#ifndef AF2_ATTN_SPLIT_MMA
#define AF2_ATTN_SPLIT_MMA 1
#endif
constexpr int ATTN_NSB = AF2_ATTN_SPLIT_MMA ? 3 : 2;
constexpr int ATTN_W_PV = ATTN_W_EPI + 4;
constexpr int ATTN_THREADS = (ATTN_W_EPI + 4 + AF2_ATTN_SPLIT_MMA) * 32;
static_assert(ATTN_W_EPI % 4 == 0, "epilogue warps must start at a multiple of 4");

template <int DH>
struct AttnSmem {
  static constexpr int Q_BYTES = 128 * DH * 2;
  static constexpr int K_BYTES = 128 * DH * 2;
  static constexpr int V_BYTES = 128 * DH * 2;
  static constexpr int BIAS_BYTES = 128 * 128 * 2;
  static constexpr int STAGE_BYTES = K_BYTES + V_BYTES + BIAS_BYTES;
  static constexpr int IDENT_BYTES = 32 * 256;
  static constexpr int Q_OFF = 0;
  static constexpr int G_OFF = 2 * Q_BYTES;
  static constexpr int KV_BYTES = K_BYTES + V_BYTES;
  static constexpr int STAGE_OFF = 4 * Q_BYTES;
  static constexpr int IDENT_OFF = STAGE_OFF + 2 * STAGE_BYTES;
  static constexpr int BAR_OFF = IDENT_OFF + IDENT_BYTES;
  static constexpr int KB_OFF = BAR_OFF + 384;
  static constexpr int MX_OFF = KB_OFF + 2 * 128 * 4;
  static constexpr int L_OFF = MX_OFF + 2 * ATTN_NSPLIT * 128 * 4;
  static constexpr int QV_OFF = L_OFF + 2 * ATTN_NSPLIT * 128 * 4;
  static constexpr int KF_OFF = QV_OFF + 2 * 128;
  static constexpr int TOTAL = KF_OFF + 16 + 1024;
};

template <int DH>
__global__ void __launch_bounds__(ATTN_THREADS, 1)
attention_tc_kernel(const __grid_constant__ CUtensorMap tmQ, const __grid_constant__ CUtensorMap tmK,
                    const __grid_constant__ CUtensorMap tmV, const __grid_constant__ CUtensorMap tmBias,
                    const __grid_constant__ CUtensorMap tmG, const __grid_constant__ CUtensorMap tmO,
                    const __grid_constant__ AttnParams p) {
  using L = AttnSmem<DH>;
  constexpr uint32_t SWZ = (DH == 64) ? SWZ_128 : SWZ_64;
  constexpr uint32_t ROWB = DH * 2;
  constexpr uint32_t SBO = 8 * ROWB;
  extern __shared__ __align__(1024) uint8_t smem[];
  if ((smem_u32(smem) & 1023u) != 0) __trap();
  uint64_t* bars = reinterpret_cast<uint64_t*>(smem + L::BAR_OFF);
  uint64_t* q_full = bars + 0;
  uint64_t* g_full = bars + 2;
  uint64_t* q_empty = bars + 4;
  uint64_t* k_full = bars + 6;
  uint64_t* k_empty = bars + 10;
  uint64_t* v_full = bars + 14;
  uint64_t* v_empty = bars + 18;
  uint64_t* s_full = bars + 40;
  uint64_t* p_full = bars + 43;
  uint64_t* kb_full = bars + 27;
  uint64_t* kb_empty = bars + 29;
  uint64_t* g_empty = bars + 31;
  uint64_t* bias_full = bars + 33;
  uint64_t* bias_empty = bars + 34;
  uint64_t* o_full = bars + 35;
  uint64_t* o_empty = bars + 37;
  uint32_t* tmem_slot = reinterpret_cast<uint32_t*>(bars + 39);
  float* keyb = reinterpret_cast<float*>(smem + L::KB_OFF);
  float* mxbuf = reinterpret_cast<float*>(smem + L::MX_OFF);
  float* lbuf = reinterpret_cast<float*>(smem + L::L_OFF);
  uint8_t* qvbuf = smem + L::QV_OFF;
  uint32_t* kflag = reinterpret_cast<uint32_t*>(smem + L::KF_OFF);

  const int warp = threadIdx.x >> 5;
  const int lane = threadIdx.x & 31;
  const int nkv = (p.n + 127) / 128;
  const int nqb = nkv;
  const int total_items = nqb * p.heads * p.nbatch;
  const bool paired = (nqb >= 2) && (nqb <= 8) && (gridDim.x % nqb == 0);
  const int n_units = paired ? p.heads * p.nbatch : total_items;
  const int n_owners = paired ? static_cast<int>(gridDim.x) / nqb : static_cast<int>(gridDim.x);
  const int owner = paired ? static_cast<int>(blockIdx.x) / nqb : static_cast<int>(blockIdx.x);
  const int item0 = static_cast<int>(static_cast<long long>(n_units) * owner / n_owners);
  const int my_items = static_cast<int>(static_cast<long long>(n_units) * (owner + 1) / n_owners) - item0;
  auto decode = [&](int it, int& qb_, int& h_, int& b_) {
    const int id = item0 + it;
    b_ = id % p.nbatch;
    if (paired) {
      qb_ = static_cast<int>(blockIdx.x) % nqb;
      h_ = id / p.nbatch;
    } else {
      qb_ = (id / p.nbatch) % nqb;
      h_ = id / (p.nbatch * nqb);
    }
  };
  auto combo_of = [&](int it) { return (item0 + it) / p.nbatch; };
  const bool resident = p.has_bias && nkv <= 2;
  const int nst = p.has_bias ? 2 : 4;
  const bool k3 = resident && p.k_stages3 != 0;
  const int nstk = k3 ? 3 : nst;
  const int stage_stride = (p.has_bias && !resident) ? L::STAGE_BYTES : L::KV_BYTES;
  auto k_off = [&](int kst) { return (k3 && kst == 2) ? (L::G_OFF + L::Q_BYTES) : (L::STAGE_OFF + kst * stage_stride); };
  auto g_slot = [&](int it) { return k3 ? 0 : (it & 1); };
  auto g_phase = [&](int it) { return static_cast<uint32_t>(k3 ? (it & 1) : ((it >> 1) & 1)); };
  const int bias_res_off = L::STAGE_OFF + 2 * L::KV_BYTES;
  constexpr uint32_t TMEM_COLS = 512;
  constexpr uint32_t S_COL = 0, O_COL = ATTN_NSB * 128;

  if (warp == 0 && lane == 0) {
    prefetch_tmap(&tmQ); prefetch_tmap(&tmK); prefetch_tmap(&tmV); prefetch_tmap(&tmG);
    if (p.has_bias) prefetch_tmap(&tmBias);
    prefetch_tmap(&tmO);
    mbar_init(bias_full, 1);
    mbar_init(bias_empty, 1);
    for (int s = 0; s < 4; ++s) {
      mbar_init(&k_full[s], 1);
      mbar_init(&k_empty[s], 1);
      mbar_init(&v_full[s], 1);
      mbar_init(&v_empty[s], 1);
    }
    for (int s = 0; s < 2; ++s) {
      mbar_init(&q_full[s], 1);
      mbar_init(&q_empty[s], 1);
      mbar_init(&o_full[s], 1);
      mbar_init(&o_empty[s], 4);
      mbar_init(&g_full[s], 1);
      mbar_init(&g_empty[s], 4);
      mbar_init(&kb_full[s], 1);
      mbar_init(&kb_empty[s], ATTN_SM_WARPS);
    }
    for (int s = 0; s < ATTN_NSB; ++s) {
      mbar_init(&s_full[s], 1);
      mbar_init(&p_full[s], ATTN_SM_WARPS);
    }
    fence_barrier_init();
  }
  if (warp == 1) tmem_alloc(tmem_slot, TMEM_COLS);
  if (p.has_bias) {
    uint4* id4 = reinterpret_cast<uint4*>(smem + L::IDENT_OFF);
    for (int i = threadIdx.x; i < L::IDENT_BYTES / 16; i += ATTN_THREADS) id4[i] = make_uint4(0u, 0u, 0u, 0u);
    __syncthreads();
    if (threadIdx.x < 16) {
      const uint32_t i = threadIdx.x, r = i & 7, c = i >> 3;
      *reinterpret_cast<__nv_bfloat16*>(smem + L::IDENT_OFF + (14 + c) * 256 + r * 32 + ((c ^ (r >> 2)) << 4) + (i & 7) * 2) =
          __float2bfloat16(1.0f);
    }
    fence_proxy_async_smem();
  }
  tc_fence_before();
  __syncthreads();
  tc_fence_after();
  const uint32_t tmem_base = *tmem_slot;
  constexpr uint32_t IDENT_COL = O_COL + 128;
  const bool ident_tmem = p.ident_tmem != 0 && ATTN_NSB == 2;
  if (p.has_bias && ident_tmem && warp >= ATTN_W_EPI && warp < ATTN_W_EPI + 4) {
    const uint32_t r = (warp & 3) * 32 + lane;
    uint32_t v[32];
#pragma unroll
    for (int half = 0; half < 2; ++half) {
#pragma unroll
      for (int c = 0; c < 32; ++c) v[c] = (static_cast<uint32_t>(half * 32 + c) == (r >> 1)) ? ((r & 1) ? 0x3f800000u : 0x00003f80u) : 0u;
      tmem_st32(tmem_base + IDENT_COL + half * 32 + (static_cast<uint32_t>((warp & 3) * 32) << 16), v);
    }
    tmem_st_wait();
    tc_fence_before();
  }
  if (p.has_bias && ident_tmem) {
    __syncthreads();
    tc_fence_after();
  }
  pdl_launch_dependents();
  pdl_wait();
  auto stamp = [&](int g, int k) {
    if (p.trace != nullptr && blockIdx.x == 0 && g < 64) p.trace[g * 16 + k] = clock64();
  };

  if (warp == 0) {
    if (lane == 0) {
      auto prefetch_block = [&](int g) {
        const int it2 = g / nkv, j2 = g - it2 * nkv;
        if (it2 >= my_items || !p.l2_prefetch) return;
        int qb2, h2, b2;
        decode(it2, qb2, h2, b2);
        tma_prefetch_4d(&tmK, 0, j2 * 128, h2, b2);
        tma_prefetch_4d(&tmV, 0, j2 * 128, h2, b2);
        if (j2 == 0) {
          tma_prefetch_4d(&tmQ, 0, qb2 * 128, h2, b2);
          tma_prefetch_4d(&tmG, 0, qb2 * 128, h2, b2);
        }
      };
      if (p.l2_prefetch) for (int g = 0; g < ATTN_PF_DIST; ++g) prefetch_block(g);
      int prev_combo = -1, nc = 0;
      int kst = 0;
      uint32_t kph = 0;
      for (int it = 0; it < my_items; ++it) {
        int qb, h, b;
        decode(it, qb, h, b);
        const int gs = it & 1;
        if (resident && combo_of(it) != prev_combo) {
          prev_combo = combo_of(it);
          mbar_wait(bias_empty, (nc & 1) ^ 1);
          mbar_arrive_expect_tx(bias_full, nkv * L::BIAS_BYTES);
          for (int j = 0; j < nkv; ++j) {
            uint8_t* sb = smem + bias_res_off + j * L::BIAS_BYTES;
            if (p.bias_t) {
              tma_load_3d(sb, &tmBias, bias_full, qb * 128, j * 128, h);
              tma_load_3d(sb + 16384, &tmBias, bias_full, qb * 128 + 64, j * 128, h);
            } else {
              tma_load_3d(sb, &tmBias, bias_full, j * 128, qb * 128, h);
              tma_load_3d(sb + 16384, &tmBias, bias_full, j * 128 + 64, qb * 128, h);
            }
          }
          ++nc;
        }
        mbar_wait(&q_empty[gs], ((it >> 1) & 1) ^ 1);
        if (p.dbg_skip & 4) mbar_arrive(&q_full[gs]);
        else {
          mbar_arrive_expect_tx(&q_full[gs], L::Q_BYTES);
          tma_load_4d(smem + L::Q_OFF + gs * L::Q_BYTES, &tmQ, &q_full[gs], 0, qb * 128, h, b);
        }
        const bool stream_bias = p.has_bias && !resident;
        for (int j = 0; j < nkv; ++j) {
          const int g = it * nkv + j;
          if (p.l2_prefetch) prefetch_block(g + ATTN_PF_DIST);
          const int ks = kst;
          mbar_wait(&k_empty[ks], kph ^ 1);
          if (++kst == nstk) { kst = 0; kph ^= 1; }
          stamp(g, 6);
          uint8_t* sk = smem + k_off(ks);
          if ((p.dbg_skip & 2) && !stream_bias) { mbar_arrive(&k_full[ks]); continue; }
          mbar_arrive_expect_tx(&k_full[ks], L::K_BYTES + (stream_bias ? L::BIAS_BYTES : 0));
          tma_load_4d(sk, &tmK, &k_full[ks], 0, j * 128, h, b);
          if (stream_bias) {
            uint8_t* sbias = sk + L::KV_BYTES;
            if (p.bias_t) {
              tma_load_3d(sbias, &tmBias, &k_full[ks], qb * 128, j * 128, h);
              tma_load_3d(sbias + 16384, &tmBias, &k_full[ks], qb * 128 + 64, j * 128, h);
            } else {
              tma_load_3d(sbias, &tmBias, &k_full[ks], j * 128, qb * 128, h);
              tma_load_3d(sbias + 16384, &tmBias, &k_full[ks], j * 128 + 64, qb * 128, h);
            }
          }
        }
      }
    }
  } else if (warp == ATTN_W_VPROD) {
    if (lane == 0) {
      int vst = 0;
      uint32_t vph = 0;
      for (int it = 0; it < my_items; ++it) {
        int qb, h, b;
        decode(it, qb, h, b);
        for (int j = 0; j < nkv; ++j) {
          const int kst = vst;
          mbar_wait(&v_empty[kst], vph ^ 1);
          if (++vst == nst) { vst = 0; vph ^= 1; }
          if (p.dbg_skip & 1) { mbar_arrive(&v_full[kst]); continue; }
          mbar_arrive_expect_tx(&v_full[kst], L::V_BYTES);
          tma_load_4d(smem + L::STAGE_OFF + kst * stage_stride + L::K_BYTES, &tmV, &v_full[kst], 0, j * 128, h, b);
        }
        if (!k3) {
          const int gs = g_slot(it);
          mbar_wait(&g_empty[gs], g_phase(it) ^ 1);
          mbar_arrive_expect_tx(&g_full[gs], L::Q_BYTES);
          tma_load_4d(smem + L::G_OFF + gs * L::Q_BYTES, &tmG, &g_full[gs], 0, qb * 128, h, b);
        }
      }
    }
  } else if (warp == 1) {
    constexpr uint32_t idesc_s = umma_idesc_bf16(128, 128, 0, 0);
    constexpr uint32_t idesc_b = umma_idesc_bf16(128, 128, 0, 1);
    constexpr uint32_t idesc_o = umma_idesc_bf16(128, DH, 0, 1);
    const int total_blocks = my_items * nkv;
    struct Walk { int g, it, j, kst, kph; };
    Walk sw = {0, 0, 0, 0, 0};
    Walk pw = {0, 0, 0, 0, 0};
    auto advance = [&](Walk& w, int depth) {
      ++w.g;
      if (++w.j == nkv) { w.j = 0; ++w.it; }
      if (++w.kst == depth) { w.kst = 0; w.kph ^= 1; }
    };
    int combo_rem = item0 % p.nbatch;
    bool combo_new = true;
    int nc = 0;
    int s_sb = 0;
    auto issue_s = [&](bool probed) {
      const int g = sw.g, it = sw.it, j = sw.j, kst = sw.kst;
      const int st = s_sb;
      if (j == 0) {
        if (!probed) mbar_wait(&q_full[it & 1], (it >> 1) & 1);
        if (resident && combo_new) {
          if (!probed) mbar_wait(bias_full, nc & 1);
          ++nc;
        }
      }
      if (lane == 0) stamp(g, 8);
      if (!probed) mbar_wait(&k_full[kst], sw.kph);
      if (lane == 0) stamp(g, 9);
      tc_fence_after();
      if (lane == 0) stamp(g, 0);
      const bool last_of_item = (j == nkv - 1);
      const bool last_of_combo = last_of_item && (it + 1 == my_items || combo_rem == p.nbatch - 1);
      if (elect_one()) {
        const uint32_t sq = smem_u32(smem + L::Q_OFF + (it & 1) * L::Q_BYTES);
        const uint32_t sk = smem_u32(smem + k_off(kst));
#pragma unroll
        for (int k = 0; k < DH / 16; ++k) {
          const uint64_t ad = umma_smem_desc(sq + k * 32, 16, SBO, SWZ);
          const uint64_t bd = umma_smem_desc(sk + k * 32, 16, SBO, SWZ);
          umma_bf16(tmem_base + S_COL + st * 128, ad, bd, idesc_s, k != 0 ? 1u : 0u);
        }
        if (p.has_bias) {
          const uint32_t si = smem_u32(smem + L::IDENT_OFF);
          const uint32_t sbz = resident ? smem_u32(smem + bias_res_off + j * L::BIAS_BYTES) : sk + L::KV_BYTES;
#pragma unroll
          for (int k = 0; k < 8; ++k) {
            const uint64_t bd = p.bias_t ? umma_smem_desc(sbz + (k >> 2) * 16384 + (k & 3) * 32, 16, 1024, SWZ_128)
                                         : umma_smem_desc(sbz + k * 2048, 16384, 1024, SWZ_128);
            const uint32_t idb = p.bias_t ? idesc_s : idesc_b;
            if (ident_tmem) {
              umma_bf16_ts(tmem_base + S_COL + st * 128, tmem_base + IDENT_COL + k * 8, bd, idb, 1u);
            } else {
              const uint64_t ad = umma_smem_desc(si + (14 - 2 * k) * 256, 16, 256, SWZ_32);
              umma_bf16(tmem_base + S_COL + st * 128, ad, bd, idb, 1u);
            }
          }
        }
        umma_commit(&s_full[st]);
        umma_commit(&k_empty[kst]);
        if (last_of_item) {
          umma_commit(&q_empty[it & 1]);
          if (resident && last_of_combo) umma_commit(bias_empty);
        }
      }
      __syncwarp();
      if (lane == 0) stamp(g, 1);
      if (last_of_item) {
        combo_new = (combo_rem == p.nbatch - 1);
        combo_rem = combo_new ? 0 : combo_rem + 1;
      } else {
        combo_new = false;
      }
      advance(sw, nstk);
      if (++s_sb == ATTN_NSB) s_sb = 0;
    };
    auto s_ready = [&]() {
      if (sw.j == 0) {
        if (!mbar_test(&q_full[sw.it & 1], (sw.it >> 1) & 1)) return false;
        if (resident && combo_new && !mbar_test(bias_full, nc & 1)) return false;
      }
      return mbar_test(&k_full[sw.kst], sw.kph);
    };
#if AF2_ATTN_SPLIT_MMA
    for (int g = 0; g < total_blocks; ++g) {
      if (g >= ATTN_NSB) {
        mbar_wait(&v_empty[pw.kst], pw.kph);
        advance(pw, nst);
      }
      issue_s(false);
    }
  } else if (warp == ATTN_W_PV) {
    constexpr uint32_t idesc_o = umma_idesc_bf16(128, DH, 0, 1);
    const int total_blocks = my_items * nkv;
    int it = 0, j = 0, vst = 0, st = 0;
    uint32_t vph = 0, sph = 0;
    for (int g = 0; g < total_blocks; ++g) {
      mbar_wait(&p_full[st], sph);
      mbar_wait(&v_full[vst], vph);
      if (j == 0) mbar_wait(&o_empty[it & 1], ((it >> 1) & 1) ^ 1);
      tc_fence_after();
      if (lane == 0) stamp(g, 2);
      if (elect_one()) {
        const uint32_t sv = smem_u32(smem + L::STAGE_OFF + vst * stage_stride + L::K_BYTES);
#pragma unroll
        for (int k = 0; k < 8; ++k) {
          const uint64_t bd = umma_smem_desc(sv + k * 2 * SBO, 16, SBO, SWZ);
          umma_bf16_ts(tmem_base + O_COL + (it & 1) * 64, tmem_base + S_COL + st * 128 + k * 8, bd, idesc_o, (j != 0 || k != 0) ? 1u : 0u);
        }
        umma_commit(&v_empty[vst]);
        if (j == nkv - 1) umma_commit(&o_full[it & 1]);
      }
      __syncwarp();
      if (lane == 0) stamp(g, 3);
      if (++j == nkv) { j = 0; ++it; }
      if (++vst == nst) { vst = 0; vph ^= 1; }
      if (++st == ATTN_NSB) { st = 0; sph ^= 1; }
    }
#else
    if (total_blocks > 0) issue_s(false);
    for (int g = 0; g < total_blocks; ++g) {
      const int st = g & 1;
      bool s_issued = g + 1 >= total_blocks;
      if (lane == 0) stamp(g + 1, 7);
      if (!s_issued && s_ready()) { issue_s(true); s_issued = true; }
      bool first = true;
      while (!mbar_test(&p_full[st], (g >> 1) & 1)) {
        if (first && lane == 0) stamp(g + 1, 10);
        first = false;
        if (!s_issued && s_ready()) { issue_s(true); s_issued = true; }
      }
      mbar_wait(&v_full[pw.kst], pw.kph);
      const int it = pw.it, j = pw.j;
      if (j == 0) mbar_wait(&o_empty[it & 1], ((it >> 1) & 1) ^ 1);
      tc_fence_after();
      if (lane == 0) stamp(g, 2);
      if (elect_one()) {
        const uint32_t sv = smem_u32(smem + L::STAGE_OFF + pw.kst * stage_stride + L::K_BYTES);
#pragma unroll
        for (int k = 0; k < 8; ++k) {
          const uint64_t bd = umma_smem_desc(sv + k * 2 * SBO, 16, SBO, SWZ);
          umma_bf16_ts(tmem_base + O_COL + (it & 1) * 64, tmem_base + S_COL + st * 128 + k * 8, bd, idesc_o, (j != 0 || k != 0) ? 1u : 0u);
        }
        umma_commit(&v_empty[pw.kst]);
        if (j == nkv - 1) umma_commit(&o_full[it & 1]);
      }
      __syncwarp();
      if (lane == 0) stamp(g, 3);
      advance(pw, nst);
      if (!s_issued) issue_s(false);
    }
#endif
  } else if (warp == ATTN_W_KEYMASK) {
    const float NEG_INF = -__int_as_float(0x7f800000);
    for (int it = 0; it < my_items; ++it) {
      int qb, h, b;
      decode(it, qb, h, b);
      for (int j = 0; j < nkv; ++j) {
        const int g = it * nkv + j;
        const int st = g & 1;
        float kb[4];
#pragma unroll
        for (int i = 0; i < 4; ++i) {
          const int kidx = j * 128 + lane * 4 + i;
          kb[i] = NEG_INF;
          if (kidx < p.n) kb[i] = (!p.mask || p.mask[b * p.mask_sb + kidx * p.mask_si]) ? 0.f : NEG_INF;
        }
        uint32_t qv = 0x01010101u;
        if (j == 0 && p.mask) {
#pragma unroll
          for (int i = 0; i < 4; ++i) {
            const int qi = qb * 128 + lane * 4 + i;
            if (qi < p.n && p.mask[b * p.mask_sb + qi * p.mask_si] == 0) qv &= ~(0xffu << (8 * i));
          }
        }
        const bool some_masked = __any_sync(0xffffffffu, (kb[0] != 0.f) | (kb[1] != 0.f) | (kb[2] != 0.f) | (kb[3] != 0.f));
        mbar_wait(&kb_empty[st], ((g >> 1) & 1) ^ 1);
        if (lane == 0) kflag[st] = some_masked ? 1u : 0u;
        *reinterpret_cast<float4*>(keyb + st * 128 + lane * 4) = make_float4(kb[0], kb[1], kb[2], kb[3]);
        if (j == 0) *reinterpret_cast<uint32_t*>(qvbuf + (it & 1) * 128 + lane * 4) = qv;
        __syncwarp();
        if (lane == 0) mbar_arrive(&kb_full[st]);
      }
    }
  } else if (warp >= ATTN_W_EPI) {
    const int q = warp & 3;
    const int r = q * 32 + lane;
    const uint32_t lane_sel = static_cast<uint32_t>(q * 32) << 16;
    for (int it = 0; it < my_items; ++it) {
      int qb, h, b;
      decode(it, qb, h, b);
      const int slot = it & 1;
      uint4 greg[DH / 8];
      if (k3) {
        const int qi = qb * 128 + r;
        const uint4* grow = reinterpret_cast<const uint4*>(p.gate + (static_cast<long long>(b) * p.tok_sb + static_cast<long long>(qi) * p.tok_si) * p.ld_gate + h * DH);
#pragma unroll
        for (int i = 0; i < DH / 8; ++i) greg[i] = (qi < p.n) ? __ldg(grow + i) : make_uint4(0u, 0u, 0u, 0u);
      }
      mbar_wait(&o_full[slot], (it >> 1) & 1);
      tc_fence_after();
      float lsum = 0.f;
#pragma unroll
      for (int i = 0; i < ATTN_NSPLIT; ++i) lsum += lbuf[(slot * ATTN_NSPLIT + i) * 128 + r];
      const float inv_l = 1.0f / lsum;
      const int gsl = g_slot(it);
      if (!k3) mbar_wait(&g_full[gsl], g_phase(it));
      uint8_t* gt = smem + L::G_OFF + gsl * L::Q_BYTES;
#pragma unroll
      for (int half = 0; half < DH / 32; ++half) {
        uint32_t o[32];
        tmem_ld32(tmem_base + O_COL + slot * 64 + half * 32 + lane_sel, o);
        tmem_ld_wait();
        if (half == DH / 32 - 1) {
          tc_fence_before();
          __syncwarp();
          if (lane == 0) mbar_arrive(&o_empty[slot]);
        }
#pragma unroll
        for (int i = 0; i < 4; ++i) {
          const uint32_t goff = (DH == 64) ? swz128_off(r, half * 4 + i) : (r * 64u + ((static_cast<uint32_t>(i) ^ ((r >> 1) & 3u)) << 4));
          const uint4 gq = k3 ? greg[half * 4 + i] : *reinterpret_cast<const uint4*>(gt + goff);
          const uint32_t gw[4] = {gq.x, gq.y, gq.z, gq.w};
          uint32_t ow[4];
#pragma unroll
          for (int t = 0; t < 4; ++t) {
            const float a = __uint_as_float(o[8 * i + 2 * t]) * inv_l * bf16lo_to_f32(gw[t]);
            const float bb = __uint_as_float(o[8 * i + 2 * t + 1]) * inv_l * bf16hi_to_f32(gw[t]);
            ow[t] = pack_bf16x2(a, bb);
          }
          *reinterpret_cast<uint4*>(gt + goff) = make_uint4(ow[0], ow[1], ow[2], ow[3]);
        }
      }
      fence_proxy_async_smem();
      __syncwarp();
      if (lane == 0) {
        if (!(p.dbg_skip & 8)) tma_store_4d(&tmO, gt + q * 32 * ROWB, 0, qb * 128 + q * 32, h, b);
        tma_store_commit();
        tma_store_wait_read<0>();
        if (!k3) mbar_arrive(&g_empty[gsl]);
      }
      __syncwarp();
    }
  } else {
    constexpr int KPT = 128 / ATTN_NSPLIT;
    const int q = warp & 3;
    const int hk = (warp - 2) >> 2;
    const int r = q * 32 + lane;
    const uint32_t lane_sel = static_cast<uint32_t>(q * 32) << 16;
    const float NEG_INF = -__int_as_float(0x7f800000);
    const bool o_owner = hk * 16 < DH;
    int sb = 0;
    uint32_t sph = 0;

    for (int it = 0; it < my_items; ++it) {
    bool q_valid = true;
    const uint32_t o_col = O_COL + (it & 1) * 64 + hk * 16;

    float m_run = NEG_INF, l_run = 0.f;
    for (int j = 0; j < nkv; ++j) {
      const int g = it * nkv + j;
      const int st = g & 1;
      mbar_wait(&kb_full[st], (g >> 1) & 1);
      if (j == 0) q_valid = qvbuf[(it & 1) * 128 + r] != 0;
      mbar_wait(&s_full[sb], sph);
      tc_fence_after();
      if (warp == 2 && lane == 0) stamp(g, 4);

      float s[KPT];
      {
        uint32_t u[KPT];
        tmem_ld32(tmem_base + S_COL + sb * 128 + hk * KPT + lane_sel, u);
        tmem_ld_wait();
#pragma unroll
        for (int i = 0; i < KPT; ++i) s[i] = __uint_as_float(u[i]);
      }
      if (kflag[st] != 0u) {
        const float* kbs = keyb + st * 128 + hk * KPT;
#pragma unroll
        for (int c = 0; c < KPT / 4; ++c) {
          const float4 k4 = *reinterpret_cast<const float4*>(kbs + c * 4);
          s[c * 4 + 0] += k4.x; s[c * 4 + 1] += k4.y; s[c * 4 + 2] += k4.z; s[c * 4 + 3] += k4.w;
        }
      }
      __syncwarp();
      if (lane == 0) mbar_arrive(&kb_empty[st]);
      if (!q_valid) {
#pragma unroll
        for (int k = 0; k < KPT; ++k) s[k] = (j * 128 + hk * KPT + k) < p.n ? 0.f : NEG_INF;
      }
      float mx0 = fmaxf(s[0], s[1]), mx1 = fmaxf(s[2], s[3]);
#pragma unroll
      for (int k = 4; k < KPT; k += 4) {
        mx0 = fmaxf(mx0, fmaxf(s[k], s[k + 1]));
        mx1 = fmaxf(mx1, fmaxf(s[k + 2], s[k + 3]));
      }
      float* mxb = mxbuf + st * ATTN_NSPLIT * 128;
      mxb[hk * 128 + r] = fmaxf(mx0, mx1);
      asm volatile("bar.sync %0, %1;" ::"r"(1 + q), "n"(32 * ATTN_NSPLIT) : "memory");
      float m_new = m_run;
#pragma unroll
      for (int i = 0; i < ATTN_NSPLIT; ++i) m_new = fmaxf(m_new, mxb[i * 128 + r]);
      bool rescale = true;
      if (j > 0) {
        rescale = __any_sync(0xffffffffu, m_new > m_run + 8.0f);
        if (!rescale) m_new = m_run;
      }
      const float m_use = (m_new == NEG_INF) ? 0.f : m_new;
      const float corr = fast_exp2(m_run - m_use);
      const f32x2 nm2 = pack2(-m_use, -m_use);
      f32x2 lsa = pack2(0.f, 0.f), lsb = pack2(0.f, 0.f);
      uint32_t pk[KPT / 2];
#pragma unroll
      for (int k = 0; k < KPT; k += 4) {
        float a0, a1, b0, b1;
        unpack2(add2(pack2(s[k], s[k + 1]), nm2), a0, a1);
        unpack2(add2(pack2(s[k + 2], s[k + 3]), nm2), b0, b1);
#if AF2_ATTN_POLY_EXP
        const float e0 = fast_exp2(a0), e2 = fast_exp2(b0);
        float e1, e3;
        unpack2(exp2_poly2(pack2(fmaxf(a1, -126.0f), fmaxf(b1, -126.0f))), e1, e3);
#else
        const float e0 = fast_exp2(a0), e1 = fast_exp2(a1), e2 = fast_exp2(b0), e3 = fast_exp2(b1);
#endif
        lsa = add2(lsa, pack2(e0, e1));
        lsb = add2(lsb, pack2(e2, e3));
        pk[k >> 1] = pack_bf16x2(e0, e1);
        pk[(k >> 1) + 1] = pack_bf16x2(e2, e3);
      }
      float ls0, ls1;
      unpack2(add2(lsa, lsb), ls0, ls1);
      l_run = l_run * corr + (ls0 + ls1);
      m_run = m_new;

      if (j > 0 && rescale) {
        mbar_wait(&v_empty[(g - 1) % nst], (((g - 1) / nst) & 1));
        tc_fence_after();
        if (o_owner) {
          uint32_t o[16];
          tmem_ld16(tmem_base + o_col + lane_sel, o);
          tmem_ld_wait();
#pragma unroll
          for (int i = 0; i < 16; ++i) o[i] = __float_as_uint(__uint_as_float(o[i]) * corr);
          tmem_st16(tmem_base + o_col + lane_sel, o);
        }
      }
      tmem_st16(tmem_base + S_COL + sb * 128 + hk * (KPT / 2) + lane_sel, pk);
      if (j == nkv - 1) {
        mbar_wait(&o_empty[it & 1], ((it >> 1) & 1) ^ 1);
        lbuf[((it & 1) * ATTN_NSPLIT + hk) * 128 + r] = l_run;
      }
      tmem_st_wait();
      tc_fence_before();
      __syncwarp();
      if (warp == 2 && lane == 0) stamp(g, 5);
      if (lane == 0) mbar_arrive(&p_full[sb]);
      if (++sb == ATTN_NSB) { sb = 0; sph ^= 1; }
    }
    }
  }

  tc_fence_before();
  __syncthreads();
  if (warp == 1) tmem_dealloc(tmem_base, TMEM_COLS);
}

}
```

Measured before the change: 4.286 million.

## Split softmax warps into two groups ping-ponging interleaved attention items

Reorganises the attention kernel so the 16 softmax warps form two groups of eight. Each group owns alternate work items and has its own S tile in TMEM. A new walk order interleaves the KV blocks of two items, so the MMA warp can issue QK^T for one item while the other group runs softmax. The O accumulator now has four slots, with per-group pv_done barriers in place of the shared split-MMA S buffers, and the identity-in-TMEM bias path is removed. Each softmax warp now covers 64 key columns in two 32-column halves, reloading logits to cut register pressure, which adds extra TMEM loads and more complex barrier and phase bookkeeping.

```diff
diff --git a/alphafold2_b200/csrc/api.cu b/alphafold2_b200/csrc/api.cu
--- a/alphafold2_b200/csrc/api.cu
+++ b/alphafold2_b200/csrc/api.cu
@@ -446,7 +446,6 @@
 
 int g_c2t_tma = 1;
 int g_attn_bias_t = 0;
-int g_attn_ident_tmem = 1;
 int g_attn_skip = 0;
 int g_attn_k3 = 0;
 int g_attn_headmajor = 0;
@@ -560,7 +559,6 @@
   p.l2_prefetch = g_attn_l2pf;
   p.k_stages3 = g_attn_k3;
   p.dbg_skip = g_attn_skip;
-  p.ident_tmem = g_attn_ident_tmem;
   p.bias_t = bias_t;
   p.trace = g_attn_trace;
   if (dh == 64) return launch_attention_inst<64>(tq, tk, tv, tb, tg, to, p, s);
@@ -733,7 +731,6 @@
   if (const char* e = getenv("AF2_ATTN_HEADMAJOR")) g_attn_headmajor = atoi(e) != 0;
   if (const char* e = getenv("AF2_ATTN_K3")) g_attn_k3 = atoi(e) != 0;
   if (const char* e = getenv("AF2_ATTN_SKIP")) g_attn_skip = atoi(e);
-  if (const char* e = getenv("AF2_ATTN_IDENT_TMEM")) g_attn_ident_tmem = atoi(e) != 0;
   if (const char* e = getenv("AF2_ATTN_BIAS_T")) g_attn_bias_t = atoi(e) != 0;
   if (const char* e = getenv("AF2_ATTN_TRACE")) {
     if (atoi(e) != 0 && !g_attn_trace) {
diff --git a/alphafold2_b200/csrc/attention_tc.cuh b/alphafold2_b200/csrc/attention_tc.cuh
--- a/alphafold2_b200/csrc/attention_tc.cuh
+++ b/alphafold2_b200/csrc/attention_tc.cuh
@@ -20,25 +20,61 @@
   long long ld_gate, ld_out;
   long long* trace;
   int bias_t;
-  int ident_tmem;
   int dbg_skip;
   int k_stages3;
   int l2_prefetch;
 };
 
 constexpr int ATTN_PF_DIST = 4;
-constexpr int ATTN_NSPLIT = 4;
-constexpr int ATTN_SM_WARPS = 4 * ATTN_NSPLIT;
+constexpr int ATTN_GROUP_WARPS = 8;
+constexpr int ATTN_NSLICE = 4;
+constexpr int ATTN_SM_WARPS = 2 * ATTN_GROUP_WARPS;
 constexpr int ATTN_W_KEYMASK = 2 + ATTN_SM_WARPS;
 constexpr int ATTN_W_VPROD = ATTN_W_KEYMASK + 1;
 constexpr int ATTN_W_EPI = ATTN_W_VPROD + 1;
-#ifndef AF2_ATTN_SPLIT_MMA
-#define AF2_ATTN_SPLIT_MMA 1
-#endif
-constexpr int ATTN_NSB = AF2_ATTN_SPLIT_MMA ? 3 : 2;
 constexpr int ATTN_W_PV = ATTN_W_EPI + 4;
-constexpr int ATTN_THREADS = (ATTN_W_EPI + 4 + AF2_ATTN_SPLIT_MMA) * 32;
+constexpr int ATTN_THREADS = (ATTN_W_PV + 1) * 32;
 static_assert(ATTN_W_EPI % 4 == 0, "epilogue warps must start at a multiple of 4");
+
+struct AttnWalk {
+  int it, j, g;
+  int base, rem;
+  bool inter;
+  int nkv, nitems, nbatch;
+  bool resident;
+  __device__ __forceinline__ AttnWalk(int nkv_, int nitems_, int nbatch_, int item0, bool resident_)
+      : it(0), j(0), g(0), base(0), rem(item0 % nbatch_), inter(false), nkv(nkv_), nitems(nitems_), nbatch(nbatch_),
+        resident(resident_) {
+    start_pair();
+  }
+  __device__ __forceinline__ bool more() const { return it < nitems; }
+  __device__ __forceinline__ void start_pair() {
+    it = base;
+    j = 0;
+    inter = base + 1 < nitems && !(resident && rem == nbatch - 1);
+  }
+  __device__ __forceinline__ void next() {
+    ++g;
+    if (inter) {
+      if (it == base) { it = base + 1; return; }
+      it = base;
+      if (++j < nkv) return;
+    } else {
+      if (++j < nkv) return;
+      if (it == base && base + 1 < nitems) { it = base + 1; j = 0; return; }
+    }
+    base += 2;
+    rem += 2;
+    if (rem >= nbatch) rem -= nbatch;
+    if (rem >= nbatch) rem -= nbatch;
+    start_pair();
+  }
+  __device__ __forceinline__ int item_rem() const { return it == base ? rem : (rem + 1 == nbatch ? 0 : rem + 1); }
+  __device__ __forceinline__ bool new_combo() const { return j == 0 && (it == 0 || item_rem() == 0); }
+  __device__ __forceinline__ bool last_of_combo() const {
+    return j == nkv - 1 && (it + 1 == nitems || item_rem() == nbatch - 1);
+  }
+};
 
 template <int DH>
 struct AttnSmem {
@@ -54,11 +90,11 @@
   static constexpr int STAGE_OFF = 4 * Q_BYTES;
   static constexpr int IDENT_OFF = STAGE_OFF + 2 * STAGE_BYTES;
   static constexpr int BAR_OFF = IDENT_OFF + IDENT_BYTES;
-  static constexpr int KB_OFF = BAR_OFF + 384;
-  static constexpr int MX_OFF = KB_OFF + 2 * 128 * 4;
-  static constexpr int L_OFF = MX_OFF + 2 * ATTN_NSPLIT * 128 * 4;
-  static constexpr int QV_OFF = L_OFF + 2 * ATTN_NSPLIT * 128 * 4;
-  static constexpr int KF_OFF = QV_OFF + 2 * 128;
+  static constexpr int KB_OFF = BAR_OFF + 512;
+  static constexpr int MX_OFF = KB_OFF + 4 * 128 * 4;
+  static constexpr int L_OFF = MX_OFF + 8 * 128 * 4;
+  static constexpr int QV_OFF = L_OFF + 4 * ATTN_NSLICE * 128 * 4;
+  static constexpr int KF_OFF = QV_OFF + 4 * 128;
   static constexpr int TOTAL = KF_OFF + 16 + 1024;
 };
 
@@ -82,16 +118,17 @@
   uint64_t* k_empty = bars + 10;
   uint64_t* v_full = bars + 14;
   uint64_t* v_empty = bars + 18;
-  uint64_t* s_full = bars + 40;
-  uint64_t* p_full = bars + 43;
-  uint64_t* kb_full = bars + 27;
-  uint64_t* kb_empty = bars + 29;
-  uint64_t* g_empty = bars + 31;
-  uint64_t* bias_full = bars + 33;
-  uint64_t* bias_empty = bars + 34;
-  uint64_t* o_full = bars + 35;
-  uint64_t* o_empty = bars + 37;
-  uint32_t* tmem_slot = reinterpret_cast<uint32_t*>(bars + 39);
+  uint64_t* s_full = bars + 22;
+  uint64_t* p_full = bars + 24;
+  uint64_t* pv_done = bars + 26;
+  uint64_t* kb_full = bars + 28;
+  uint64_t* kb_empty = bars + 32;
+  uint64_t* g_empty = bars + 36;
+  uint64_t* bias_full = bars + 38;
+  uint64_t* bias_empty = bars + 39;
+  uint64_t* o_full = bars + 40;
+  uint64_t* o_empty = bars + 44;
+  uint32_t* tmem_slot = reinterpret_cast<uint32_t*>(bars + 48);
   float* keyb = reinterpret_cast<float*>(smem + L::KB_OFF);
   float* mxbuf = reinterpret_cast<float*>(smem + L::MX_OFF);
   float* lbuf = reinterpret_cast<float*>(smem + L::L_OFF);
@@ -120,8 +157,9 @@
       h_ = id / (p.nbatch * nqb);
     }
   };
-  auto combo_of = [&](int it) { return (item0 + it) / p.nbatch; };
   const bool resident = p.has_bias && nkv <= 2;
+  auto walk = [&]() { return AttnWalk(nkv, my_items, p.nbatch, item0, resident); };
+  auto o_slot = [](int it) { return (it & 1) * 2 + ((it >> 1) & 1); };
   const int nst = p.has_bias ? 2 : 4;
   const bool k3 = resident && p.k_stages3 != 0;
   const int nstk = k3 ? 3 : nst;
@@ -131,7 +169,7 @@
   auto g_phase = [&](int it) { return static_cast<uint32_t>(k3 ? (it & 1) : ((it >> 1) & 1)); };
   const int bias_res_off = L::STAGE_OFF + 2 * L::KV_BYTES;
   constexpr uint32_t TMEM_COLS = 512;
-  constexpr uint32_t S_COL = 0, O_COL = ATTN_NSB * 128;
+  constexpr uint32_t O_COL = 256;
 
   if (warp == 0 && lane == 0) {
     prefetch_tmap(&tmQ); prefetch_tmap(&tmK); prefetch_tmap(&tmV); prefetch_tmap(&tmG);
@@ -144,20 +182,19 @@
       mbar_init(&k_empty[s], 1);
       mbar_init(&v_full[s], 1);
       mbar_init(&v_empty[s], 1);
+      mbar_init(&o_full[s], 1);
+      mbar_init(&o_empty[s], 4);
+      mbar_init(&kb_full[s], 1);
+      mbar_init(&kb_empty[s], ATTN_GROUP_WARPS);
     }
     for (int s = 0; s < 2; ++s) {
       mbar_init(&q_full[s], 1);
       mbar_init(&q_empty[s], 1);
-      mbar_init(&o_full[s], 1);
-      mbar_init(&o_empty[s], 4);
       mbar_init(&g_full[s], 1);
       mbar_init(&g_empty[s], 4);
-      mbar_init(&kb_full[s], 1);
-      mbar_init(&kb_empty[s], ATTN_SM_WARPS);
-    }
-    for (int s = 0; s < ATTN_NSB; ++s) {
       mbar_init(&s_full[s], 1);
-      mbar_init(&p_full[s], ATTN_SM_WARPS);
+      mbar_init(&p_full[s], ATTN_GROUP_WARPS);
+      mbar_init(&pv_done[s], 1);
     }
     fence_barrier_init();
   }
@@ -177,24 +214,6 @@
   __syncthreads();
   tc_fence_after();
   const uint32_t tmem_base = *tmem_slot;
-  constexpr uint32_t IDENT_COL = O_COL + 128;
-  const bool ident_tmem = p.ident_tmem != 0 && ATTN_NSB == 2;
-  if (p.has_bias && ident_tmem && warp >= ATTN_W_EPI && warp < ATTN_W_EPI + 4) {
-    const uint32_t r = (warp & 3) * 32 + lane;
-    uint32_t v[32];
-#pragma unroll
-    for (int half = 0; half < 2; ++half) {
-#pragma unroll
-      for (int c = 0; c < 32; ++c) v[c] = (static_cast<uint32_t>(half * 32 + c) == (r >> 1)) ? ((r & 1) ? 0x3f800000u : 0x00003f80u) : 0u;
-      tmem_st32(tmem_base + IDENT_COL + half * 32 + (static_cast<uint32_t>((warp & 3) * 32) << 16), v);
-    }
-    tmem_st_wait();
-    tc_fence_before();
-  }
-  if (p.has_bias && ident_tmem) {
-    __syncthreads();
-    tc_fence_after();
-  }
   pdl_launch_dependents();
   pdl_wait();
   auto stamp = [&](int g, int k) {
@@ -216,56 +235,55 @@
         }
       };
       if (p.l2_prefetch) for (int g = 0; g < ATTN_PF_DIST; ++g) prefetch_block(g);
-      int prev_combo = -1, nc = 0;
+      int nc = 0;
       int kst = 0;
       uint32_t kph = 0;
-      for (int it = 0; it < my_items; ++it) {
+      const bool stream_bias = p.has_bias && !resident;
+      for (AttnWalk w = walk(); w.more(); w.next()) {
+        const int it = w.it, j = w.j;
         int qb, h, b;
         decode(it, qb, h, b);
-        const int gs = it & 1;
-        if (resident && combo_of(it) != prev_combo) {
-          prev_combo = combo_of(it);
-          mbar_wait(bias_empty, (nc & 1) ^ 1);
-          mbar_arrive_expect_tx(bias_full, nkv * L::BIAS_BYTES);
-          for (int j = 0; j < nkv; ++j) {
-            uint8_t* sb = smem + bias_res_off + j * L::BIAS_BYTES;
-            if (p.bias_t) {
-              tma_load_3d(sb, &tmBias, bias_full, qb * 128, j * 128, h);
-              tma_load_3d(sb + 16384, &tmBias, bias_full, qb * 128 + 64, j * 128, h);
-            } else {
-              tma_load_3d(sb, &tmBias, bias_full, j * 128, qb * 128, h);
-              tma_load_3d(sb + 16384, &tmBias, bias_full, j * 128 + 64, qb * 128, h);
+        if (j == 0) {
+          if (resident && w.new_combo()) {
+            mbar_wait(bias_empty, (nc & 1) ^ 1);
+            mbar_arrive_expect_tx(bias_full, nkv * L::BIAS_BYTES);
+            for (int jj = 0; jj < nkv; ++jj) {
+              uint8_t* sb = smem + bias_res_off + jj * L::BIAS_BYTES;
+              if (p.bias_t) {
+                tma_load_3d(sb, &tmBias, bias_full, qb * 128, jj * 128, h);
+                tma_load_3d(sb + 16384, &tmBias, bias_full, qb * 128 + 64, jj * 128, h);
+              } else {
+                tma_load_3d(sb, &tmBias, bias_full, jj * 128, qb * 128, h);
+                tma_load_3d(sb + 16384, &tmBias, bias_full, jj * 128 + 64, qb * 128, h);
+              }
             }
+            ++nc;
           }
-          ++nc;
-        }
-        mbar_wait(&q_empty[gs], ((it >> 1) & 1) ^ 1);
-        if (p.dbg_skip & 4) mbar_arrive(&q_full[gs]);
-        else {
-          mbar_arrive_expect_tx(&q_full[gs], L::Q_BYTES);
-          tma_load_4d(smem + L::Q_OFF + gs * L::Q_BYTES, &tmQ, &q_full[gs], 0, qb * 128, h, b);
-        }
-        const bool stream_bias = p.has_bias && !resident;
-        for (int j = 0; j < nkv; ++j) {
-          const int g = it * nkv + j;
-          if (p.l2_prefetch) prefetch_block(g + ATTN_PF_DIST);
-          const int ks = kst;
-          mbar_wait(&k_empty[ks], kph ^ 1);
-          if (++kst == nstk) { kst = 0; kph ^= 1; }
-          stamp(g, 6);
-          uint8_t* sk = smem + k_off(ks);
-          if ((p.dbg_skip & 2) && !stream_bias) { mbar_arrive(&k_full[ks]); continue; }
-          mbar_arrive_expect_tx(&k_full[ks], L::K_BYTES + (stream_bias ? L::BIAS_BYTES : 0));
-          tma_load_4d(sk, &tmK, &k_full[ks], 0, j * 128, h, b);
-          if (stream_bias) {
-            uint8_t* sbias = sk + L::KV_BYTES;
-            if (p.bias_t) {
-              tma_load_3d(sbias, &tmBias, &k_full[ks], qb * 128, j * 128, h);
-              tma_load_3d(sbias + 16384, &tmBias, &k_full[ks], qb * 128 + 64, j * 128, h);
-            } else {
-              tma_load_3d(sbias, &tmBias, &k_full[ks], j * 128, qb * 128, h);
-              tma_load_3d(sbias + 16384, &tmBias, &k_full[ks], j * 128 + 64, qb * 128, h);
-            }
+          const int gs = it & 1;
+          mbar_wait(&q_empty[gs], ((it >> 1) & 1) ^ 1);
+          if (p.dbg_skip & 4) mbar_arrive(&q_full[gs]);
+          else {
+            mbar_arrive_expect_tx(&q_full[gs], L::Q_BYTES);
+            tma_load_4d(smem + L::Q_OFF + gs * L::Q_BYTES, &tmQ, &q_full[gs], 0, qb * 128, h, b);
+          }
+        }
+        if (p.l2_prefetch) prefetch_block(it * nkv + j + ATTN_PF_DIST);
+        const int ks = kst;
+        mbar_wait(&k_empty[ks], kph ^ 1);
+        if (++kst == nstk) { kst = 0; kph ^= 1; }
+        stamp(w.g, 6);
+        uint8_t* sk = smem + k_off(ks);
+        if ((p.dbg_skip & 2) && !stream_bias) { mbar_arrive(&k_full[ks]); continue; }
+        mbar_arrive_expect_tx(&k_full[ks], L::K_BYTES + (stream_bias ? L::BIAS_BYTES : 0));
+        tma_load_4d(sk, &tmK, &k_full[ks], 0, j * 128, h, b);
+        if (stream_bias) {
+          uint8_t* sbias = sk + L::KV_BYTES;
+          if (p.bias_t) {
+            tma_load_3d(sbias, &tmBias, &k_full[ks], qb * 128, j * 128, h);
+            tma_load_3d(sbias + 16384, &tmBias, &k_full[ks], qb * 128 + 64, j * 128, h);
+          } else {
+            tma_load_3d(sbias, &tmBias, &k_full[ks], j * 128, qb * 128, h);
+            tma_load_3d(sbias + 16384, &tmBias, &k_full[ks], j * 128 + 64, qb * 128, h);
           }
         }
       }
@@ -274,18 +292,19 @@
     if (lane == 0) {
       int vst = 0;
       uint32_t vph = 0;
-      for (int it = 0; it < my_items; ++it) {
+      for (AttnWalk w = walk(); w.more(); w.next()) {
+        const int it = w.it, j = w.j;
         int qb, h, b;
         decode(it, qb, h, b);
-        for (int j = 0; j < nkv; ++j) {
-          const int kst = vst;
-          mbar_wait(&v_empty[kst], vph ^ 1);
-          if (++vst == nst) { vst = 0; vph ^= 1; }
-          if (p.dbg_skip & 1) { mbar_arrive(&v_full[kst]); continue; }
+        const int kst = vst;
+        mbar_wait(&v_empty[kst], vph ^ 1);
+        if (++vst == nst) { vst = 0; vph ^= 1; }
+        if (p.dbg_skip & 1) mbar_arrive(&v_full[kst]);
+        else {
           mbar_arrive_expect_tx(&v_full[kst], L::V_BYTES);
           tma_load_4d(smem + L::STAGE_OFF + kst * stage_stride + L::K_BYTES, &tmV, &v_full[kst], 0, j * 128, h, b);
         }
-        if (!k3) {
+        if (j == nkv - 1 && !k3) {
           const int gs = g_slot(it);
           mbar_wait(&g_empty[gs], g_phase(it) ^ 1);
           mbar_arrive_expect_tx(&g_full[gs], L::Q_BYTES);
@@ -296,45 +315,40 @@
   } else if (warp == 1) {
     constexpr uint32_t idesc_s = umma_idesc_bf16(128, 128, 0, 0);
     constexpr uint32_t idesc_b = umma_idesc_bf16(128, 128, 0, 1);
-    constexpr uint32_t idesc_o = umma_idesc_bf16(128, DH, 0, 1);
-    const int total_blocks = my_items * nkv;
-    struct Walk { int g, it, j, kst, kph; };
-    Walk sw = {0, 0, 0, 0, 0};
-    Walk pw = {0, 0, 0, 0, 0};
-    auto advance = [&](Walk& w, int depth) {
-      ++w.g;
-      if (++w.j == nkv) { w.j = 0; ++w.it; }
-      if (++w.kst == depth) { w.kst = 0; w.kph ^= 1; }
-    };
-    int combo_rem = item0 % p.nbatch;
-    bool combo_new = true;
-    int nc = 0;
-    int s_sb = 0;
-    auto issue_s = [&](bool probed) {
-      const int g = sw.g, it = sw.it, j = sw.j, kst = sw.kst;
-      const int st = s_sb;
+    int nc = 0, kst = 0;
+    uint32_t kph = 0;
+    uint32_t started = 0, pv_ph = 0;
+    for (AttnWalk w = walk(); w.more(); w.next()) {
+      const int g = w.g, it = w.it, j = w.j, grp = it & 1;
+      if ((started >> grp) & 1u) {
+        mbar_wait(&pv_done[grp], (pv_ph >> grp) & 1u);
+        pv_ph ^= 1u << grp;
+      }
+      started |= 1u << grp;
       if (j == 0) {
-        if (!probed) mbar_wait(&q_full[it & 1], (it >> 1) & 1);
-        if (resident && combo_new) {
-          if (!probed) mbar_wait(bias_full, nc & 1);
+        mbar_wait(&q_full[grp], (it >> 1) & 1);
+        if (resident && w.new_combo()) {
+          mbar_wait(bias_full, nc & 1);
           ++nc;
         }
       }
       if (lane == 0) stamp(g, 8);
-      if (!probed) mbar_wait(&k_full[kst], sw.kph);
-      if (lane == 0) stamp(g, 9);
+      mbar_wait(&k_full[kst], kph);
+      if (lane == 0) {
+        stamp(g, 9);
+        if (p.trace != nullptr && blockIdx.x == 0 && g < 64) p.trace[g * 16 + 11] = 1 + grp;
+      }
       tc_fence_after();
       if (lane == 0) stamp(g, 0);
-      const bool last_of_item = (j == nkv - 1);
-      const bool last_of_combo = last_of_item && (it + 1 == my_items || combo_rem == p.nbatch - 1);
+      const uint32_t s_tm = tmem_base + grp * 128;
       if (elect_one()) {
-        const uint32_t sq = smem_u32(smem + L::Q_OFF + (it & 1) * L::Q_BYTES);
+        const uint32_t sq = smem_u32(smem + L::Q_OFF + grp * L::Q_BYTES);
         const uint32_t sk = smem_u32(smem + k_off(kst));
 #pragma unroll
         for (int k = 0; k < DH / 16; ++k) {
           const uint64_t ad = umma_smem_desc(sq + k * 32, 16, SBO, SWZ);
           const uint64_t bd = umma_smem_desc(sk + k * 32, 16, SBO, SWZ);
-          umma_bf16(tmem_base + S_COL + st * 128, ad, bd, idesc_s, k != 0 ? 1u : 0u);
+          umma_bf16(s_tm, ad, bd, idesc_s, k != 0 ? 1u : 0u);
         }
         if (p.has_bias) {
           const uint32_t si = smem_u32(smem + L::IDENT_OFF);
@@ -344,56 +358,31 @@
             const uint64_t bd = p.bias_t ? umma_smem_desc(sbz + (k >> 2) * 16384 + (k & 3) * 32, 16, 1024, SWZ_128)
                                          : umma_smem_desc(sbz + k * 2048, 16384, 1024, SWZ_128);
             const uint32_t idb = p.bias_t ? idesc_s : idesc_b;
-            if (ident_tmem) {
-              umma_bf16_ts(tmem_base + S_COL + st * 128, tmem_base + IDENT_COL + k * 8, bd, idb, 1u);
-            } else {
-              const uint64_t ad = umma_smem_desc(si + (14 - 2 * k) * 256, 16, 256, SWZ_32);
-              umma_bf16(tmem_base + S_COL + st * 128, ad, bd, idb, 1u);
-            }
+            const uint64_t ad = umma_smem_desc(si + (14 - 2 * k) * 256, 16, 256, SWZ_32);
+            umma_bf16(s_tm, ad, bd, idb, 1u);
           }
         }
-        umma_commit(&s_full[st]);
+        umma_commit(&s_full[grp]);
         umma_commit(&k_empty[kst]);
-        if (last_of_item) {
-          umma_commit(&q_empty[it & 1]);
-          if (resident && last_of_combo) umma_commit(bias_empty);
+        if (j == nkv - 1) {
+          umma_commit(&q_empty[grp]);
+          if (resident && w.last_of_combo()) umma_commit(bias_empty);
         }
       }
       __syncwarp();
       if (lane == 0) stamp(g, 1);
-      if (last_of_item) {
-        combo_new = (combo_rem == p.nbatch - 1);
-        combo_rem = combo_new ? 0 : combo_rem + 1;
-      } else {
-        combo_new = false;
-      }
-      advance(sw, nstk);
-      if (++s_sb == ATTN_NSB) s_sb = 0;
-    };
-    auto s_ready = [&]() {
-      if (sw.j == 0) {
-        if (!mbar_test(&q_full[sw.it & 1], (sw.it >> 1) & 1)) return false;
-        if (resident && combo_new && !mbar_test(bias_full, nc & 1)) return false;
-      }
-      return mbar_test(&k_full[sw.kst], sw.kph);
-    };
-#if AF2_ATTN_SPLIT_MMA
-    for (int g = 0; g < total_blocks; ++g) {
-      if (g >= ATTN_NSB) {
-        mbar_wait(&v_empty[pw.kst], pw.kph);
-        advance(pw, nst);
-      }
-      issue_s(false);
+      if (++kst == nstk) { kst = 0; kph ^= 1; }
     }
   } else if (warp == ATTN_W_PV) {
     constexpr uint32_t idesc_o = umma_idesc_bf16(128, DH, 0, 1);
-    const int total_blocks = my_items * nkv;
-    int it = 0, j = 0, vst = 0, st = 0;
-    uint32_t vph = 0, sph = 0;
-    for (int g = 0; g < total_blocks; ++g) {
-      mbar_wait(&p_full[st], sph);
+    int vst = 0;
+    uint32_t vph = 0, p_ph = 0;
+    for (AttnWalk w = walk(); w.more(); w.next()) {
+      const int g = w.g, it = w.it, j = w.j, grp = it & 1, os = o_slot(it);
+      mbar_wait(&p_full[grp], (p_ph >> grp) & 1u);
+      p_ph ^= 1u << grp;
       mbar_wait(&v_full[vst], vph);
-      if (j == 0) mbar_wait(&o_empty[it & 1], ((it >> 1) & 1) ^ 1);
+      if (j == 0) mbar_wait(&o_empty[os], ((it >> 2) & 1) ^ 1);
       tc_fence_after();
       if (lane == 0) stamp(g, 2);
       if (elect_one()) {
@@ -401,82 +390,48 @@
 #pragma unroll
         for (int k = 0; k < 8; ++k) {
           const uint64_t bd = umma_smem_desc(sv + k * 2 * SBO, 16, SBO, SWZ);
-          umma_bf16_ts(tmem_base + O_COL + (it & 1) * 64, tmem_base + S_COL + st * 128 + k * 8, bd, idesc_o, (j != 0 || k != 0) ? 1u : 0u);
+          umma_bf16_ts(tmem_base + O_COL + os * 64, tmem_base + grp * 128 + (k >> 1) * 32 + (k & 1) * 8, bd, idesc_o,
+                       (j != 0 || k != 0) ? 1u : 0u);
         }
         umma_commit(&v_empty[vst]);
-        if (j == nkv - 1) umma_commit(&o_full[it & 1]);
+        umma_commit(&pv_done[grp]);
+        if (j == nkv - 1) umma_commit(&o_full[os]);
       }
       __syncwarp();
       if (lane == 0) stamp(g, 3);
-      if (++j == nkv) { j = 0; ++it; }
       if (++vst == nst) { vst = 0; vph ^= 1; }
-      if (++st == ATTN_NSB) { st = 0; sph ^= 1; }
-    }
-#else
-    if (total_blocks > 0) issue_s(false);
-    for (int g = 0; g < total_blocks; ++g) {
-      const int st = g & 1;
-      bool s_issued = g + 1 >= total_blocks;
-      if (lane == 0) stamp(g + 1, 7);
-      if (!s_issued && s_ready()) { issue_s(true); s_issued = true; }
-      bool first = true;
-      while (!mbar_test(&p_full[st], (g >> 1) & 1)) {
-        if (first && lane == 0) stamp(g + 1, 10);
-        first = false;
-        if (!s_issued && s_ready()) { issue_s(true); s_issued = true; }
-      }
-      mbar_wait(&v_full[pw.kst], pw.kph);
-      const int it = pw.it, j = pw.j;
-      if (j == 0) mbar_wait(&o_empty[it & 1], ((it >> 1) & 1) ^ 1);
-      tc_fence_after();
-      if (lane == 0) stamp(g, 2);
-      if (elect_one()) {
-        const uint32_t sv = smem_u32(smem + L::STAGE_OFF + pw.kst * stage_stride + L::K_BYTES);
-#pragma unroll
-        for (int k = 0; k < 8; ++k) {
-          const uint64_t bd = umma_smem_desc(sv + k * 2 * SBO, 16, SBO, SWZ);
-          umma_bf16_ts(tmem_base + O_COL + (it & 1) * 64, tmem_base + S_COL + st * 128 + k * 8, bd, idesc_o, (j != 0 || k != 0) ? 1u : 0u);
-        }
-        umma_commit(&v_empty[pw.kst]);
-        if (j == nkv - 1) umma_commit(&o_full[it & 1]);
-      }
-      __syncwarp();
-      if (lane == 0) stamp(g, 3);
-      advance(pw, nst);
-      if (!s_issued) issue_s(false);
-    }
-#endif
+    }
   } else if (warp == ATTN_W_KEYMASK) {
     const float NEG_INF = -__int_as_float(0x7f800000);
-    for (int it = 0; it < my_items; ++it) {
+    int cnt0 = 0, cnt1 = 0;
+    for (AttnWalk w = walk(); w.more(); w.next()) {
+      const int it = w.it, j = w.j, grp = it & 1;
       int qb, h, b;
       decode(it, qb, h, b);
-      for (int j = 0; j < nkv; ++j) {
-        const int g = it * nkv + j;
-        const int st = g & 1;
-        float kb[4];
+      const int c = grp ? cnt1++ : cnt0++;
+      const int st = grp * 2 + (c & 1);
+      float kb[4];
+#pragma unroll
+      for (int i = 0; i < 4; ++i) {
+        const int kidx = j * 128 + lane * 4 + i;
+        kb[i] = NEG_INF;
+        if (kidx < p.n) kb[i] = (!p.mask || p.mask[b * p.mask_sb + kidx * p.mask_si]) ? 0.f : NEG_INF;
+      }
+      uint32_t qv = 0x01010101u;
+      if (j == 0 && p.mask) {
 #pragma unroll
         for (int i = 0; i < 4; ++i) {
-          const int kidx = j * 128 + lane * 4 + i;
-          kb[i] = NEG_INF;
-          if (kidx < p.n) kb[i] = (!p.mask || p.mask[b * p.mask_sb + kidx * p.mask_si]) ? 0.f : NEG_INF;
-        }
-        uint32_t qv = 0x01010101u;
-        if (j == 0 && p.mask) {
-#pragma unroll
-          for (int i = 0; i < 4; ++i) {
-            const int qi = qb * 128 + lane * 4 + i;
-            if (qi < p.n && p.mask[b * p.mask_sb + qi * p.mask_si] == 0) qv &= ~(0xffu << (8 * i));
-          }
-        }
-        const bool some_masked = __any_sync(0xffffffffu, (kb[0] != 0.f) | (kb[1] != 0.f) | (kb[2] != 0.f) | (kb[3] != 0.f));
-        mbar_wait(&kb_empty[st], ((g >> 1) & 1) ^ 1);
-        if (lane == 0) kflag[st] = some_masked ? 1u : 0u;
-        *reinterpret_cast<float4*>(keyb + st * 128 + lane * 4) = make_float4(kb[0], kb[1], kb[2], kb[3]);
-        if (j == 0) *reinterpret_cast<uint32_t*>(qvbuf + (it & 1) * 128 + lane * 4) = qv;
-        __syncwarp();
-        if (lane == 0) mbar_arrive(&kb_full[st]);
-      }
+          const int qi = qb * 128 + lane * 4 + i;
+          if (qi < p.n && p.mask[b * p.mask_sb + qi * p.mask_si] == 0) qv &= ~(0xffu << (8 * i));
+        }
+      }
+      const bool some_masked = __any_sync(0xffffffffu, (kb[0] != 0.f) | (kb[1] != 0.f) | (kb[2] != 0.f) | (kb[3] != 0.f));
+      mbar_wait(&kb_empty[st], ((c >> 1) & 1) ^ 1);
+      if (lane == 0) kflag[st] = some_masked ? 1u : 0u;
+      *reinterpret_cast<float4*>(keyb + st * 128 + lane * 4) = make_float4(kb[0], kb[1], kb[2], kb[3]);
+      if (j == 0) *reinterpret_cast<uint32_t*>(qvbuf + st * 128 + lane * 4) = qv;
+      __syncwarp();
+      if (lane == 0) mbar_arrive(&kb_full[st]);
     }
   } else if (warp >= ATTN_W_EPI) {
     const int q = warp & 3;
@@ -485,7 +440,7 @@
     for (int it = 0; it < my_items; ++it) {
       int qb, h, b;
       decode(it, qb, h, b);
-      const int slot = it & 1;
+      const int os = o_slot(it);
       uint4 greg[DH / 8];
       if (k3) {
         const int qi = qb * 128 + r;
@@ -493,11 +448,11 @@
 #pragma unroll
         for (int i = 0; i < DH / 8; ++i) greg[i] = (qi < p.n) ? __ldg(grow + i) : make_uint4(0u, 0u, 0u, 0u);
       }
-      mbar_wait(&o_full[slot], (it >> 1) & 1);
+      mbar_wait(&o_full[os], (it >> 2) & 1);
       tc_fence_after();
       float lsum = 0.f;
 #pragma unroll
-      for (int i = 0; i < ATTN_NSPLIT; ++i) lsum += lbuf[(slot * ATTN_NSPLIT + i) * 128 + r];
+      for (int i = 0; i < ATTN_NSLICE; ++i) lsum += lbuf[(os * ATTN_NSLICE + i) * 128 + r];
       const float inv_l = 1.0f / lsum;
       const int gsl = g_slot(it);
       if (!k3) mbar_wait(&g_full[gsl], g_phase(it));
@@ -505,12 +460,12 @@
 #pragma unroll
       for (int half = 0; half < DH / 32; ++half) {
         uint32_t o[32];
-        tmem_ld32(tmem_base + O_COL + slot * 64 + half * 32 + lane_sel, o);
+        tmem_ld32(tmem_base + O_COL + os * 64 + half * 32 + lane_sel, o);
         tmem_ld_wait();
         if (half == DH / 32 - 1) {
           tc_fence_before();
           __syncwarp();
-          if (lane == 0) mbar_arrive(&o_empty[slot]);
+          if (lane == 0) mbar_arrive(&o_empty[os]);
         }
 #pragma unroll
         for (int i = 0; i < 4; ++i) {
@@ -538,64 +493,76 @@
       __syncwarp();
     }
   } else {
-    constexpr int KPT = 128 / ATTN_NSPLIT;
+    const int grp = (warp - 2) / ATTN_GROUP_WARPS;
+    const int hk = ((warp - 2) >> 2) & 1;
     const int q = warp & 3;
-    const int hk = (warp - 2) >> 2;
     const int r = q * 32 + lane;
     const uint32_t lane_sel = static_cast<uint32_t>(q * 32) << 16;
+    const uint32_t s_tm = tmem_base + grp * 128 + hk * 64 + lane_sel;
+    const bool tracer = ((warp - 2) % ATTN_GROUP_WARPS) == 0 && lane == 0;
     const float NEG_INF = -__int_as_float(0x7f800000);
-    const bool o_owner = hk * 16 < DH;
-    int sb = 0;
-    uint32_t sph = 0;
-
-    for (int it = 0; it < my_items; ++it) {
+    auto stream_pos = [&](int it, int j) {
+      const int base = it & ~1;
+      const bool inter = base + 1 < my_items && !(resident && (item0 + base) % p.nbatch == p.nbatch - 1);
+      return base * nkv + (inter ? 2 * j + (it & 1) : (it & 1) * nkv + j);
+    };
+    int cnt = 0;
     bool q_valid = true;
-    const uint32_t o_col = O_COL + (it & 1) * 64 + hk * 16;
-
-    float m_run = NEG_INF, l_run = 0.f;
+    float m_run = NEG_INF, l_lo = 0.f, l_hi = 0.f;
+
+    for (int it = grp; it < my_items; it += 2)
     for (int j = 0; j < nkv; ++j) {
-      const int g = it * nkv + j;
-      const int st = g & 1;
-      mbar_wait(&kb_full[st], (g >> 1) & 1);
-      if (j == 0) q_valid = qvbuf[(it & 1) * 128 + r] != 0;
-      mbar_wait(&s_full[sb], sph);
+      const int st = grp * 2 + (cnt & 1);
+      const uint32_t ph = cnt & 1;
+      mbar_wait(&kb_full[st], (cnt >> 1) & 1);
+      if (j == 0) {
+        q_valid = qvbuf[st * 128 + r] != 0;
+        m_run = NEG_INF;
+        l_lo = 0.f;
+        l_hi = 0.f;
+      }
+      mbar_wait(&s_full[grp], ph);
       tc_fence_after();
-      if (warp == 2 && lane == 0) stamp(g, 4);
-
-      float s[KPT];
-      {
-        uint32_t u[KPT];
-        tmem_ld32(tmem_base + S_COL + sb * 128 + hk * KPT + lane_sel, u);
+      if (tracer) stamp(stream_pos(it, j), 4);
+      const bool kmasked = kflag[st] != 0u;
+      auto logits = [&](int hf, float (&s)[32]) {
+        uint32_t u[32];
+        tmem_ld32(s_tm + hf * 32, u);
         tmem_ld_wait();
 #pragma unroll
-        for (int i = 0; i < KPT; ++i) s[i] = __uint_as_float(u[i]);
-      }
-      if (kflag[st] != 0u) {
-        const float* kbs = keyb + st * 128 + hk * KPT;
-#pragma unroll
-        for (int c = 0; c < KPT / 4; ++c) {
-          const float4 k4 = *reinterpret_cast<const float4*>(kbs + c * 4);
-          s[c * 4 + 0] += k4.x; s[c * 4 + 1] += k4.y; s[c * 4 + 2] += k4.z; s[c * 4 + 3] += k4.w;
-        }
-      }
-      __syncwarp();
-      if (lane == 0) mbar_arrive(&kb_empty[st]);
-      if (!q_valid) {
-#pragma unroll
-        for (int k = 0; k < KPT; ++k) s[k] = (j * 128 + hk * KPT + k) < p.n ? 0.f : NEG_INF;
-      }
-      float mx0 = fmaxf(s[0], s[1]), mx1 = fmaxf(s[2], s[3]);
-#pragma unroll
-      for (int k = 4; k < KPT; k += 4) {
-        mx0 = fmaxf(mx0, fmaxf(s[k], s[k + 1]));
-        mx1 = fmaxf(mx1, fmaxf(s[k + 2], s[k + 3]));
-      }
-      float* mxb = mxbuf + st * ATTN_NSPLIT * 128;
-      mxb[hk * 128 + r] = fmaxf(mx0, mx1);
-      asm volatile("bar.sync %0, %1;" ::"r"(1 + q), "n"(32 * ATTN_NSPLIT) : "memory");
-      float m_new = m_run;
-#pragma unroll
-      for (int i = 0; i < ATTN_NSPLIT; ++i) m_new = fmaxf(m_new, mxb[i * 128 + r]);
+        for (int i = 0; i < 32; ++i) s[i] = __uint_as_float(u[i]);
+        if (kmasked) {
+          const float* kbs = keyb + st * 128 + hk * 64 + hf * 32;
+#pragma unroll
+          for (int c = 0; c < 8; ++c) {
+            const float4 k4 = *reinterpret_cast<const float4*>(kbs + c * 4);
+            s[c * 4 + 0] += k4.x; s[c * 4 + 1] += k4.y; s[c * 4 + 2] += k4.z; s[c * 4 + 3] += k4.w;
+          }
+        }
+        if (!q_valid) {
+#pragma unroll
+          for (int k = 0; k < 32; ++k) s[k] = (j * 128 + hk * 64 + hf * 32 + k) < p.n ? 0.f : NEG_INF;
+        }
+      };
+      auto slice_max = [](const float (&s)[32]) {
+        float mx0 = fmaxf(s[0], s[1]), mx1 = fmaxf(s[2], s[3]);
+#pragma unroll
+        for (int k = 4; k < 32; k += 4) {
+          mx0 = fmaxf(mx0, fmaxf(s[k], s[k + 1]));
+          mx1 = fmaxf(mx1, fmaxf(s[k + 2], s[k + 3]));
+        }
+        return fmaxf(mx0, mx1);
+      };
+      float s[32];
+      logits(0, s);
+      float mx = slice_max(s);
+      logits(1, s);
+      mx = fmaxf(mx, slice_max(s));
+      float* mxb = mxbuf + (grp * 2 + ph) * 2 * 128;
+      mxb[hk * 128 + r] = mx;
+      asm volatile("bar.sync %0, %1;" ::"r"(1 + grp * 4 + q), "n"(64) : "memory");
+      float m_new = fmaxf(m_run, mxb[r]);
+      m_new = fmaxf(m_new, mxb[128 + r]);
       bool rescale = true;
       if (j > 0) {
         rescale = __any_sync(0xffffffffu, m_new > m_run + 8.0f);
@@ -604,54 +571,64 @@
       const float m_use = (m_new == NEG_INF) ? 0.f : m_new;
       const float corr = fast_exp2(m_run - m_use);
       const f32x2 nm2 = pack2(-m_use, -m_use);
-      f32x2 lsa = pack2(0.f, 0.f), lsb = pack2(0.f, 0.f);
-      uint32_t pk[KPT / 2];
-#pragma unroll
-      for (int k = 0; k < KPT; k += 4) {
-        float a0, a1, b0, b1;
-        unpack2(add2(pack2(s[k], s[k + 1]), nm2), a0, a1);
-        unpack2(add2(pack2(s[k + 2], s[k + 3]), nm2), b0, b1);
+      auto exp_store = [&](int hf, const float (&s)[32], float& l_run) {
+        f32x2 lsa = pack2(0.f, 0.f), lsb = pack2(0.f, 0.f);
+        uint32_t pk[16];
+#pragma unroll
+        for (int k = 0; k < 32; k += 4) {
+          float a0, a1, b0, b1;
+          unpack2(add2(pack2(s[k], s[k + 1]), nm2), a0, a1);
+          unpack2(add2(pack2(s[k + 2], s[k + 3]), nm2), b0, b1);
 #if AF2_ATTN_POLY_EXP
-        const float e0 = fast_exp2(a0), e2 = fast_exp2(b0);
-        float e1, e3;
-        unpack2(exp2_poly2(pack2(fmaxf(a1, -126.0f), fmaxf(b1, -126.0f))), e1, e3);
+          const float e0 = fast_exp2(a0), e2 = fast_exp2(b0);
+          float e1, e3;
+          unpack2(exp2_poly2(pack2(fmaxf(a1, -126.0f), fmaxf(b1, -126.0f))), e1, e3);
 #else
-        const float e0 = fast_exp2(a0), e1 = fast_exp2(a1), e2 = fast_exp2(b0), e3 = fast_exp2(b1);
+          const float e0 = fast_exp2(a0), e1 = fast_exp2(a1), e2 = fast_exp2(b0), e3 = fast_exp2(b1);
 #endif
-        lsa = add2(lsa, pack2(e0, e1));
-        lsb = add2(lsb, pack2(e2, e3));
-        pk[k >> 1] = pack_bf16x2(e0, e1);
-        pk[(k >> 1) + 1] = pack_bf16x2(e2, e3);
-      }
-      float ls0, ls1;
-      unpack2(add2(lsa, lsb), ls0, ls1);
-      l_run = l_run * corr + (ls0 + ls1);
+          lsa = add2(lsa, pack2(e0, e1));
+          lsb = add2(lsb, pack2(e2, e3));
+          pk[k >> 1] = pack_bf16x2(e0, e1);
+          pk[(k >> 1) + 1] = pack_bf16x2(e2, e3);
+        }
+        float ls0, ls1;
+        unpack2(add2(lsa, lsb), ls0, ls1);
+        l_run = l_run * corr + (ls0 + ls1);
+        tmem_st16(s_tm + hf * 32, pk);
+      };
+      exp_store(1, s, l_hi);
+      logits(0, s);
+      exp_store(0, s, l_lo);
+      __syncwarp();
+      if (lane == 0) mbar_arrive(&kb_empty[st]);
       m_run = m_new;
 
       if (j > 0 && rescale) {
-        mbar_wait(&v_empty[(g - 1) % nst], (((g - 1) / nst) & 1));
+        mbar_wait(&pv_done[grp], (cnt - 1) & 1);
         tc_fence_after();
-        if (o_owner) {
+        const uint32_t o_tm = tmem_base + O_COL + o_slot(it) * 64 + hk * (DH / 2) + lane_sel;
+#pragma unroll
+        for (int c = 0; c < DH / 32; ++c) {
           uint32_t o[16];
-          tmem_ld16(tmem_base + o_col + lane_sel, o);
+          tmem_ld16(o_tm + c * 16, o);
           tmem_ld_wait();
 #pragma unroll
           for (int i = 0; i < 16; ++i) o[i] = __float_as_uint(__uint_as_float(o[i]) * corr);
-          tmem_st16(tmem_base + o_col + lane_sel, o);
-        }
-      }
-      tmem_st16(tmem_base + S_COL + sb * 128 + hk * (KPT / 2) + lane_sel, pk);
+          tmem_st16(o_tm + c * 16, o);
+        }
+      }
       if (j == nkv - 1) {
-        mbar_wait(&o_empty[it & 1], ((it >> 1) & 1) ^ 1);
-        lbuf[((it & 1) * ATTN_NSPLIT + hk) * 128 + r] = l_run;
+        const int os = o_slot(it);
+        mbar_wait(&o_empty[os], ((it >> 2) & 1) ^ 1);
+        lbuf[(os * ATTN_NSLICE + 2 * hk) * 128 + r] = l_lo;
+        lbuf[(os * ATTN_NSLICE + 2 * hk + 1) * 128 + r] = l_hi;
       }
       tmem_st_wait();
       tc_fence_before();
       __syncwarp();
-      if (warp == 2 && lane == 0) stamp(g, 5);
-      if (lane == 0) mbar_arrive(&p_full[sb]);
-      if (++sb == ATTN_NSB) { sb = 0; sph ^= 1; }
-    }
+      if (tracer) stamp(stream_pos(it, j), 5);
+      if (lane == 0) mbar_arrive(&p_full[grp]);
+      ++cnt;
     }
   }
 
```

Result: slower. 4.025 million, median of 6 (-6.1%).
